# danielSanchezQ/dkg

Measured on AMD Instinct MI355X. Metric: verified shares/sec (whole node) at n=1024,t=511; full-ceremony wall time, higher is better.
Workload: dtype u32 (GF(2^255-19), Z_l); 1 GPU; one DKG ceremony n=1024, t=511 (share gen + round-2/4 checks + finalise); n=1024, t=511, parallelism=single GPU, verify_streams=2, rounds_2_4_fused=True, degree_split=4, recombination=short lattice multipliers, recombination_addends=affine Niels, stepping_additions=dedicated (complete redo where exceptional)

## Files before the change

dkg_amd/_lib.py:

```python
import ctypes
import os
import sys

HERE = os.path.dirname(os.path.abspath(__file__))
LIB_PATH = os.environ.get("DKG_AMD_LIB", os.path.join(HERE, "libdkg_amd.so"))

DKG_OK = 0
DKG_E_ARG = -1
DKG_E_DECODE = -2
DKG_E_DEVICE = -3
DKG_E_NOMEM = -4
REJECT, ACCEPT, SELF, SKIPPED, MISSING = 0, 1, 2, 3, 4
FIN_OK, FIN_R2_ERROR, FIN_R4_ERROR, FIN_PHASE4_ERROR, FIN_INSUFFICIENT, FIN_PANIC = 0, 1, 2, 3, 4, 5
COMPLAINT_IGNORED, COMPLAINT_NO_PHASE3 = 4, 5

_lib = None


class DkgError(RuntimeError):
    def __init__(self, code, msg=""):
        self.code = code
        names = {DKG_E_ARG: "DKG_E_ARG", DKG_E_DECODE: "DKG_E_DECODE", DKG_E_DEVICE: "DKG_E_DEVICE",
                 DKG_E_NOMEM: "DKG_E_NOMEM"}
        super().__init__(f"{names.get(code, code)}: {msg}")


class CeremonyOut(ctypes.Structure):
    _fields_ = [
        ("E", ctypes.c_void_p), ("A", ctypes.c_void_p),
        ("s", ctypes.c_void_p), ("s_prime", ctypes.c_void_p),
        ("dec2", ctypes.c_void_p), ("dec4", ctypes.c_void_p),
        ("qualified", ctypes.c_void_p), ("r2_error", ctypes.c_void_p), ("r4_error", ctypes.c_void_p),
        ("complaints2", ctypes.c_void_p), ("reconstruct", ctypes.c_void_p),
        ("final_share", ctypes.c_void_p), ("public_share", ctypes.c_void_p),
        ("mpk", ctypes.c_uint8 * 32),
        ("n_qualified", ctypes.c_int32), ("phase4_error", ctypes.c_int32),
        ("ms_round1", ctypes.c_double), ("ms_round2", ctypes.c_double), ("ms_round3", ctypes.c_double),
        ("ms_round4", ctypes.c_double), ("ms_finalise", ctypes.c_double), ("ms_total", ctypes.c_double),
    ]


class ShardOutcome(ctypes.Structure):
    _fields_ = [
        ("qualified", ctypes.c_void_p), ("complaints2", ctypes.c_void_p), ("r2_error", ctypes.c_void_p),
        ("reconstruct", ctypes.c_void_p), ("r4_error", ctypes.c_void_p),
        ("n_qualified", ctypes.c_int32), ("phase4_error", ctypes.c_int32),
    ]


class BatchOut(ctypes.Structure):
    _fields_ = [
        ("mpk", ctypes.c_void_p), ("n_qualified", ctypes.c_void_p), ("phase4_error", ctypes.c_void_p),
        ("qualified", ctypes.c_void_p),
        ("r2_error", ctypes.c_void_p), ("r4_error", ctypes.c_void_p), ("complaints2", ctypes.c_void_p),
        ("reconstruct", ctypes.c_void_p), ("final_share", ctypes.c_void_p), ("public_share", ctypes.c_void_p),
        ("dec2", ctypes.c_void_p), ("dec4", ctypes.c_void_p),
        ("ms_round1", ctypes.c_double), ("ms_checks", ctypes.c_double), ("ms_round3", ctypes.c_double),
        ("ms_finalise", ctypes.c_double), ("ms_total", ctypes.c_double),
    ]


def lib():
    global _lib
    if _lib is not None:
        return _lib
    if not os.path.exists(LIB_PATH):
        raise RuntimeError(f"{LIB_PATH} is missing: build it with `make -C dkg_amd` or __graft_entry__.build()")
    if "torch" not in sys.modules and not os.environ.get("DKG_NO_TORCH_PREIMPORT"):
        try:
            import torch
        except Exception:
            pass
    L = ctypes.CDLL(LIB_PATH)
    sz, p, u8p = ctypes.c_size_t, ctypes.c_void_p, ctypes.c_char_p
    L.dkg_ctx_create.argtypes = [ctypes.c_int, ctypes.POINTER(p)]
    L.dkg_ctx_destroy.argtypes = [p]
    L.dkg_ctx_destroy.restype = None
    L.dkg_ctx_last_error.argtypes = [p]
    L.dkg_ctx_last_error.restype = ctypes.c_char_p
    L.dkg_device_count.argtypes = []
    L.dkg_ctx_set_streams.argtypes = [p, ctypes.c_int]
    L.dkg_ctx_set_overlap.argtypes = [p, ctypes.c_int]
    L.dkg_ctx_set_verify_mode.argtypes = [p, ctypes.c_int]
    L.dkg_ctx_fallback_rows.argtypes = [p]
    L.dkg_ctx_fallback_rows.restype = sz
    L.dkg_ctx_set_split.argtypes = [p, ctypes.c_int]
    L.dkg_ctx_set_stepping.argtypes = [p, ctypes.c_int]
    L.dkg_ctx_set_field_mode.argtypes = [p, ctypes.c_int]
    L.dkg_ctx_set_binomial.argtypes = [p, ctypes.c_int]
    L.dkg_ctx_set_check.argtypes = [p, ctypes.c_int]
    L.dkg_ctx_last_split.argtypes = [p]
    L.dkg_ctx_last_split_len.argtypes = [p]
    L.dkg_ctx_last_split_len.restype = sz
    L.dkg_split_model_ms.argtypes = [sz, sz, sz, ctypes.c_int]
    L.dkg_split_model_ms.restype = ctypes.c_double
    L.dkg_split_len.argtypes = [sz, sz, sz, ctypes.c_int]
    L.dkg_split_len.restype = sz
    L.dkg_ctx_set_combine.argtypes = [p, ctypes.c_int]
    L.dkg_ctx_last_combine.argtypes = [p]
    L.dkg_ctx_last_binomial.argtypes = [p]
    L.dkg_ctx_set_addends.argtypes = [p, ctypes.c_int]
    L.dkg_ctx_set_stepping_formula.argtypes = [p, ctypes.c_int]
    L.dkg_ctx_stepping_redos.argtypes = [p]
    L.dkg_ctx_stepping_redos.restype = ctypes.c_longlong
    L.dkg_ctx_binomial_reruns.argtypes = [p]
    L.dkg_ctx_clock_probe.argtypes = [p, ctypes.c_uint, ctypes.POINTER(ctypes.c_double), ctypes.POINTER(ctypes.c_double)]
    L.dkg_device_pci_bus_id.argtypes = [ctypes.c_int, ctypes.c_char_p, ctypes.c_int]
    L.dkg_split_multipliers.argtypes = [sz, sz, ctypes.c_int, p, p]
    L.dkg_ctx_phase_ms.argtypes = [p, ctypes.c_char_p]
    L.dkg_ctx_phase_ms.restype = ctypes.c_double
    L.dkg_env_check.argtypes = [sz, sz]
    L.dkg_env_init.argtypes = [p, sz, sz, u8p, sz, p]
    L.dkg_msm_batch.argtypes = [p, sz, sz, u8p, u8p, p]
    L.dkg_fixed_base_batch.argtypes = [p, p, sz, u8p, p]
    L.dkg_poly_eval_batch.argtypes = [p, sz, sz, u8p, sz, p, p]
    L.dkg_points_valid_batch.argtypes = [p, sz, u8p, p]
    L.dkg_share_gen.argtypes = [p, sz, sz, sz, u8p, u8p, p, p, p, p]
    L.dkg_verify_pairs.argtypes = [p, sz, sz, ctypes.c_int, sz, sz, u8p, u8p, p, p]
    L.dkg_verify_receiver.argtypes = [p, sz, sz, ctypes.c_int, sz, u8p, u8p, p, p]
    L.dkg_ceremony_run.argtypes = [p, sz, sz, u8p, u8p, ctypes.POINTER(CeremonyOut)]
    L.dkg_ceremony_verify.argtypes = [p, sz, sz, u8p, u8p, u8p, u8p, ctypes.POINTER(CeremonyOut)]
    L.dkg_ceremony_verify_fetched.argtypes = [p, sz, sz, u8p, u8p, u8p, u8p, u8p, u8p, ctypes.POINTER(CeremonyOut)]
    L.dkg_ceremony_run_device.argtypes = [p, sz, sz, p, p, ctypes.POINTER(CeremonyOut)]
    L.dkg_ceremony_shard_device.argtypes = [p, sz, sz, sz, sz, p, p, p, p, p, p, ctypes.POINTER(ctypes.c_double)]
    L.dkg_ceremony_shard_verify_device.argtypes = [p, sz, sz, sz, sz, p, p, p, p, p, p, p, p,
                                                    ctypes.POINTER(ctypes.c_double)]
    L.dkg_ceremony_batch_device.argtypes = [p, sz, sz, sz, p, p, ctypes.POINTER(BatchOut)]
    L.dkg_ceremony_batch_verify.argtypes = [p, sz, sz, sz, u8p, u8p, u8p, u8p, ctypes.POINTER(BatchOut)]
    L.dkg_dealer_coeffs_device.argtypes = [p, u8p, ctypes.c_uint32, sz, sz, sz, sz, p, p]
    L.dkg_member_keys.argtypes = [p, u8p, ctypes.c_uint32, sz, p, p]
    L.dkg_enc_randomness.argtypes = [u8p, ctypes.c_uint32, sz, sz, sz, sz, p]
    L.dkg_enc_randomness_device.argtypes = [p, u8p, ctypes.c_uint32, sz, sz, sz, sz, sz, p]
    L.dkg_encrypt_shares.argtypes = [p, sz, sz, u8p, u8p, u8p, u8p, p, p]
    L.dkg_decrypt_shares.argtypes = [p, sz, sz, u8p, u8p, u8p, p, p, p]
    L.dkg_ceremony_run_full_device.argtypes = [p, sz, sz, p, p, p, u8p, u8p, ctypes.POINTER(CeremonyOut)]
    L.dkg_ceremony_verify_full.argtypes = [p, sz, sz, u8p, u8p, u8p, u8p, u8p, ctypes.POINTER(CeremonyOut)]
    L.dkg_member_keys_batch.argtypes = [p, u8p, ctypes.c_uint32, sz, sz, p, p]
    L.dkg_encrypt_shares_batch.argtypes = [p, sz, sz, u8p, u8p, u8p, u8p, p, p]
    L.dkg_decrypt_shares_batch.argtypes = [p, sz, sz, u8p, u8p, u8p, p, p, p]
    L.dkg_ceremony_batch_full_device.argtypes = [p, sz, sz, sz, p, p, p, u8p, u8p, ctypes.POINTER(BatchOut)]
    L.dkg_ceremony_batch_verify_full.argtypes = [p, sz, sz, sz, u8p, u8p, u8p, u8p, u8p, ctypes.POINTER(BatchOut),
                                                 p, p]
    L.dkg_ctx_set_batch_full_chunk.argtypes = [p, sz]
    L.dkg_misbehaviour_prove.argtypes = [p, sz, u8p, u8p, u8p, p]
    L.dkg_complaint1_verify.argtypes = [p, sz, sz, p, u8p, u8p, u8p, u8p, p]
    L.dkg_complaint3_verify.argtypes = [p, sz, sz, p, u8p, u8p, u8p, u8p, p]
    L.dkg_complaints_prove.argtypes = [p, sz, u8p, u8p, u8p, p]
    L.dkg_complaints_verify.argtypes = [p, sz, sz, sz, p, p, u8p, u8p, u8p, u8p, u8p, p, p]
    L.dkg_ctx_set_complaint_eval.argtypes = [p, ctypes.c_int]
    L.dkg_ceremony_verify_full_complaints.argtypes = [p, sz, sz, u8p, u8p, u8p, u8p, u8p, u8p, sz, p, p, u8p,
                                                      ctypes.POINTER(CeremonyOut), p, p]
    L.dkg_complaints3_verify.argtypes = [p, sz, sz, sz, p, p, u8p, u8p, u8p, u8p, u8p, u8p, p, p]
    L.dkg_ceremony_verify_fetched_proven.argtypes = [p, sz, sz, u8p, u8p, u8p, u8p, u8p, u8p, sz, p, p, u8p, u8p,
                                                     ctypes.POINTER(CeremonyOut), p, p, p]
    L.dkg_ceremony_verify_full_proven.argtypes = [p, sz, sz, u8p, u8p, u8p, u8p, u8p, u8p, sz, p, p, u8p, u8p, sz, p, p,
                                                  u8p, u8p, ctypes.POINTER(CeremonyOut), p, p, p, p, p]
    L.dkg_dealer_coeffs.argtypes = [u8p, ctypes.c_uint32, sz, sz, sz, p, p]
    L.dkg_scalar_sum_device.argtypes = [p, sz, sz, p, p, p]
    L.dkg_point_sum_device.argtypes = [p, sz, p, p, p]
    L.dkg_share_gen_device.argtypes = [p, sz, sz, sz, p, p, p, p, p, p]
    L.dkg_ceremony_shard_recon_device.argtypes = [p, sz, sz, sz, sz, u8p, u8p, u8p, u8p, p, p,
                                                  ctypes.POINTER(ctypes.c_int32)]
    L.dkg_finalise_parties.argtypes = [p, sz, sz, u8p, u8p, u8p, u8p, u8p, u8p, u8p, p, p, p]
    L.dkg_shard_range.argtypes = [sz, sz, sz, ctypes.POINTER(sz), ctypes.POINTER(sz)]
    L.dkg_shard_range.restype = None
    L.dkg_shard_rows.argtypes = [sz, sz]
    L.dkg_shard_rows.restype = sz
    L.dkg_shard_combine_device.argtypes = [p, sz, sz, sz, p, p, p, p, ctypes.POINTER(ShardOutcome)]
    L.dkg_shard_combine_packed_device.argtypes = [p, sz, sz, sz, p, p, p, p, ctypes.POINTER(ShardOutcome)]
    L.dkg_fixed_base_windows.argtypes = []
    L.dkg_key_comb_windows.argtypes = []
    L.dkg_packed_row_words.argtypes = [sz]
    L.dkg_packed_row_words.restype = sz
    L.dkg_decisions_pack_device.argtypes = [p, sz, sz, sz, sz, p, p]
    L.dkg_shard_finalise_device.argtypes = [p, sz, sz, sz, p, p, u8p, ctypes.c_int, p, p, p]
    L.dkg_multi_create.argtypes = [ctypes.POINTER(ctypes.c_int), ctypes.c_int, ctypes.POINTER(p)]
    L.dkg_multi_destroy.argtypes = [p]
    L.dkg_multi_destroy.restype = None
    L.dkg_multi_size.argtypes = [p]
    L.dkg_multi_ctx.argtypes = [p, ctypes.c_int]
    L.dkg_multi_ctx.restype = p
    L.dkg_multi_last_error.argtypes = [p]
    L.dkg_multi_last_error.restype = ctypes.c_char_p
    L.dkg_multi_phase_ms.argtypes = [p, ctypes.c_char_p]
    L.dkg_multi_phase_ms.restype = ctypes.c_double
    L.dkg_multi_env_init.argtypes = [p, sz, sz, u8p, sz, p]
    L.dkg_multi_ceremony_run.argtypes = [p, sz, sz, u8p, u8p, ctypes.POINTER(CeremonyOut)]
    L.dkg_multi_ceremony_run_device.argtypes = [p, sz, sz, ctypes.POINTER(p), ctypes.POINTER(p),
                                                ctypes.POINTER(CeremonyOut)]
    L.dkg_multi_ceremony_verify.argtypes = [p, sz, sz, u8p, u8p, u8p, u8p, ctypes.POINTER(CeremonyOut)]
    _lib = L
    return L


EXPORTED = [
    "dkg_ctx_create", "dkg_ctx_destroy", "dkg_ctx_last_error", "dkg_ctx_phase_ms", "dkg_ctx_set_streams", "dkg_ctx_set_overlap",
    "dkg_device_count", "dkg_env_init",
    "dkg_env_check", "dkg_msm_batch", "dkg_fixed_base_batch", "dkg_poly_eval_batch",
    "dkg_points_valid_batch", "dkg_share_gen", "dkg_verify_pairs", "dkg_verify_receiver",
    "dkg_ctx_set_split", "dkg_ctx_set_stepping", "dkg_ctx_set_field_mode", "dkg_ctx_set_binomial", "dkg_ctx_set_check", "dkg_ctx_last_split", "dkg_ctx_last_split_len", "dkg_ctx_set_verify_mode", "dkg_ctx_fallback_rows", "dkg_split_model_ms", "dkg_split_len",
    "dkg_ctx_set_combine", "dkg_ctx_last_combine", "dkg_ctx_last_binomial", "dkg_ctx_set_addends", "dkg_ctx_set_stepping_formula", "dkg_ctx_stepping_redos", "dkg_ctx_binomial_reruns", "dkg_split_multipliers",
    "dkg_ctx_clock_probe", "dkg_device_pci_bus_id",
    "dkg_ceremony_run", "dkg_ceremony_verify", "dkg_ceremony_verify_fetched", "dkg_ceremony_run_device", "dkg_ceremony_shard_device",
    "dkg_ceremony_shard_verify_device",
    "dkg_ceremony_batch_device", "dkg_ceremony_batch_verify", "dkg_member_keys", "dkg_enc_randomness",
    "dkg_enc_randomness_device", "dkg_encrypt_shares", "dkg_decrypt_shares", "dkg_ceremony_run_full_device",
    "dkg_ceremony_verify_full", "dkg_misbehaviour_prove", "dkg_complaint1_verify", "dkg_complaint3_verify", "dkg_dealer_coeffs", "dkg_dealer_coeffs_device",
    "dkg_scalar_sum_device", "dkg_point_sum_device", "dkg_ceremony_shard_recon_device", "dkg_finalise_parties",
    "dkg_share_gen_device", "dkg_shard_range", "dkg_shard_rows", "dkg_shard_combine_device",
    "dkg_shard_combine_packed_device", "dkg_packed_row_words", "dkg_fixed_base_windows", "dkg_key_comb_windows", "dkg_decisions_pack_device",
    "dkg_shard_finalise_device", "dkg_multi_create", "dkg_multi_destroy", "dkg_multi_size", "dkg_multi_ctx",
    "dkg_multi_last_error", "dkg_multi_phase_ms", "dkg_multi_env_init", "dkg_multi_ceremony_run",
    "dkg_multi_ceremony_run_device", "dkg_multi_ceremony_verify",
    "dkg_member_keys_batch", "dkg_encrypt_shares_batch", "dkg_decrypt_shares_batch", "dkg_ceremony_batch_full_device",
    "dkg_ceremony_batch_verify_full", "dkg_ctx_set_batch_full_chunk",
    "dkg_complaints_prove", "dkg_complaints_verify", "dkg_ctx_set_complaint_eval", "dkg_ceremony_verify_full_complaints",
    "dkg_complaints3_verify", "dkg_ceremony_verify_fetched_proven", "dkg_ceremony_verify_full_proven",
]
```

dkg_amd/csrc/ge25519.h:

```cpp
#pragma once
#include "fe25519.h"

struct ge_p3 {
  fe X, Y, Z, T;
};
struct ge_cached {
  fe YpX, YmX, Z2, T2d;
};
struct ge_aff {
  fe ypx, ymx, xy2d;
};

namespace ge_const {
__device__ static const uint32_t D[10] = {0x35978a3u, 0xd37284u, 0x3156ebdu, 0x6a0a0eu, 0x1c029u,
                                          0x179e898u, 0x3a03cbbu, 0x1ce7198u, 0x2e2b6ffu, 0x1480db3u};
__device__ static const uint32_t D2[10] = {0x2b2f159u, 0x1a6e509u, 0x22add7au, 0xd4141du, 0x38052u,
                                           0xf3d130u, 0x3407977u, 0x19ce331u, 0x1c56dffu, 0x901b67u};
__device__ static const uint32_t SQRT_M1[10] = {0x20ea0b0u, 0x186c9d2u, 0x8f189du, 0x35697fu,
                                                0xbd0c60u, 0x1fbd7a7u, 0x2804c9eu, 0x1e16569u,
                                                0x4fc1du, 0xae0c92u};
__device__ static const uint32_t SQRT_AD_MINUS_ONE[10] = {
    0x17b2e1bu, 0x1fda812u, 0x297afd2u, 0x60dbc2u, 0x2be7638u,
    0x1f5d1fdu, 0x27e6498u, 0x11581e7u, 0x3f2b834u, 0xdda4c6u};
__device__ static const uint32_t INVSQRT_A_MINUS_D[10] = {
// ... 150 lines not shown
    fe_dbl(c, c);
    fe_add(h, a, b);
    fe_sub(e, h, t);
    fe_sub(g, a, b);
    fe_add(f, c, g);
    fe_carry(f, f);
    fe_mul2(r.X, e, f, r.Y, g, h);
    if (with_t) fe_mul2(r.Z, g, f, r.T, e, h);
    else fe_mul(r.Z, g, f);
    return;
  }
  fe a, b, c, e, f, g, h, t;
  fe_sq(a, p.X);
  fe_sq(b, p.Y);
  fe_sq(c, p.Z);
  fe_dbl(c, c);
  fe_add(t, p.X, p.Y);
  fe_sq(t, t);
  fe_add(h, a, b);
  fe_sub(e, h, t);
  fe_sub(g, a, b);
  fe_add(f, c, g);
  fe_carry(f, f);
  fe_mul(r.X, e, f);
  fe_mul(r.Y, g, h);
  fe_mul(r.Z, g, f);
  if (with_t) fe_mul(r.T, e, h);
}

template <bool IL = false>
DKG_DEV void ge_dbl_rt(ge_p3& r, const ge_p3& p, bool with_t) {
  if constexpr (IL && DKG_PW) {
    fe a, b, c, t, h, e, g;
    fe_add(t, p.X, p.Y);
    fe_sq2(a, p.X, b, p.Y);
    fe_sq2(c, p.Z, t, t);
    fe_dbl(c, c);
    fe_add(h, a, b);
    fe_sub(e, h, t);
    fe_sub(g, a, b);
    fe_add(c, c, g);
    fe_carry(c, c);
    fe_mul2(r.X, e, c, r.Y, g, h);
    if (with_t) fe_mul2(r.Z, g, c, r.T, e, h);
    else fe_mul(r.Z, g, c);
    return;
  }
  fe a, b, c, t, h, e, g;
  fe_sq(a, p.X);
  fe_sq(b, p.Y);
  fe_sq(c, p.Z);
  fe_dbl(c, c);
  fe_add(t, p.X, p.Y);
  fe_sq(t, t);
  fe_add(h, a, b);
  fe_sub(e, h, t);
  fe_sub(g, a, b);
  fe_add(c, c, g);
  fe_carry(c, c);
  fe_mul(r.X, e, c);
  fe_mul(r.Y, g, h);
  fe_mul(r.Z, g, c);
  if (with_t) fe_mul(r.T, e, h);
}

template <bool IL = false>
DKG_DEV void ge_dbl_lean(ge_p3& r, const ge_p3& p, bool with_t) {
  if constexpr (IL && DKG_PW) {
    fe a, b, t, h, g;
    fe_sq2(a, p.X, b, p.Y);
    fe_add(h, a, b);
    fe_sub(g, a, b);
    fe_add(a, p.X, p.Y);
    fe_sq2(t, p.Z, a, a);
    fe_dbl(t, t);
    fe_add(t, t, g);
    fe_carry(t, t);
    fe_sub(b, h, a);
    fe_mul2(r.X, b, t, r.Y, g, h);
    if (with_t) fe_mul2(r.Z, g, t, r.T, b, h);
    else fe_mul(r.Z, g, t);
    return;
  }
  fe a, b, t, h, g;
  fe_sq(a, p.X);
  fe_sq(b, p.Y);
  fe_add(h, a, b);
  fe_sub(g, a, b);
  fe_sq(t, p.Z);
  fe_dbl(t, t);
  fe_add(t, t, g);
  fe_carry(t, t);
  fe_add(a, p.X, p.Y);
  fe_sq(a, a);
  fe_sub(b, h, a);
  fe_mul(r.X, b, t);
  fe_mul(r.Y, g, h);
  fe_mul(r.Z, g, t);
  if (with_t) fe_mul(r.T, b, h);
}

template <bool IL = false>
DKG_DEV void ge_add_signed(ge_p3& r, const ge_p3& p, const ge_cached& q, bool neg, bool with_t = true) {
  fe a, b, e, h, t, qa, qb;
#pragma unroll
  for (int i = 0; i < 10; i++) {
    qa.v[i] = neg ? q.YpX.v[i] : q.YmX.v[i];
    qb.v[i] = neg ? q.YmX.v[i] : q.YpX.v[i];
  }
  if constexpr (IL && DKG_PW) {
    fe u;
    fe_sub(t, p.Y, p.X);
    fe_add(u, p.Y, p.X);
    fe_mul2(a, t, qa, b, u, qb);
  } else {
    fe_sub(t, p.Y, p.X);
    fe_mul(a, t, qa);
    fe_add(t, p.Y, p.X);
    fe_mul(b, t, qb);
  }
  fe_sub(e, b, a);
  fe_add(h, b, a);
  if constexpr (IL && DKG_PW) {
    fe_mul2(a, p.T, q.T2d, b, p.Z, q.Z2);
  } else {
    fe_mul(a, p.T, q.T2d);
    fe_mul(b, p.Z, q.Z2);
  }
  fe na;
  fe_neg(na, a);
  fe_cmov(a, na, neg);
  fe_sub(t, b, a);
  fe_add(b, b, a);
  if constexpr (IL && DKG_PW) {
    fe_mul2(r.X, e, t, r.Y, b, h);
    if (with_t) fe_mul2(r.Z, b, t, r.T, e, h);
    else fe_mul(r.Z, b, t);
  } else {
    fe_mul(r.X, e, t);
    fe_mul(r.Y, b, h);
    fe_mul(r.Z, b, t);
    if (with_t) fe_mul(r.T, e, h);
  }
}

template <bool IL = false>
DKG_DEV void ge_madd_signed(ge_p3& r, const ge_p3& p, const ge_aff& q, bool neg, bool with_t = true) {
  fe a, b, e, h, t, qa, qb;
#pragma unroll
  for (int i = 0; i < 10; i++) {
    qa.v[i] = neg ? q.ypx.v[i] : q.ymx.v[i];
    qb.v[i] = neg ? q.ymx.v[i] : q.ypx.v[i];
  }
  if constexpr (IL && DKG_PW) {
    fe u;
    fe_sub(t, p.Y, p.X);
    fe_add(u, p.Y, p.X);
    fe_mul2(a, t, qa, b, u, qb);
  } else {
    fe_sub(t, p.Y, p.X);
    fe_mul(a, t, qa);
    fe_add(t, p.Y, p.X);
    fe_mul(b, t, qb);
  }
  fe_sub(e, b, a);
  fe_add(h, b, a);
  fe_mul(a, p.T, q.xy2d);
  fe na;
  fe_neg(na, a);
  fe_cmov(a, na, neg);
  fe_dbl(b, p.Z);
  fe_carry(b, b);
  fe_sub(t, b, a);
  fe_add(b, b, a);
  if constexpr (IL && DKG_PW) {
    fe_mul2(r.X, e, t, r.Y, b, h);
    if (with_t) fe_mul2(r.Z, b, t, r.T, e, h);
    else fe_mul(r.Z, b, t);
  } else {
    fe_mul(r.X, e, t);
    fe_mul(r.Y, b, h);
    fe_mul(r.Z, b, t);
    if (with_t) fe_mul(r.T, e, h);
  }
}


DKG_DEV bool fe_sqrt_ratio_m1(fe& r, const fe& u, const fe& v) {
  fe v3, v7, t, chk, neg_u, neg_u_i, sqrtm1;
  fe_ld(sqrtm1, ge_const::SQRT_M1);
  fe_sq(v3, v);
  fe_mul(v3, v3, v);
  fe_sq(v7, v3);
  fe_mul(v7, v7, v);
  fe_mul(t, u, v7);
  fe_pow22523(t, t);
  fe_mul(t, t, v3);
  fe_mul(r, t, u);
  fe_sq(chk, r);
  fe_mul(chk, chk, v);
  fe_neg(neg_u, u);
  fe_carry(neg_u, neg_u);
  fe_mul(neg_u_i, neg_u, sqrtm1);
  fe d;
  fe_sub(d, chk, u);
  bool correct = fe_iszero(d);
  fe_sub(d, chk, neg_u);
  bool flipped = fe_iszero(d);
  fe_sub(d, chk, neg_u_i);
  bool flipped_i = fe_iszero(d);
  fe r_prime;
  fe_mul(r_prime, r, sqrtm1);
  fe_cmov(r, r_prime, flipped || flipped_i);
  fe_abs(r, r);
  return correct || flipped;
}

DKG_DEV void fe_sq_x2(fe (&r)[2], const fe (&a)[2]) { fe_sq2(r[0], a[0], r[1], a[1]); }
DKG_DEV void fe_mul_x2(fe (&r)[2], const fe (&a)[2], const fe (&b)[2]) {
  fe_mul2(r[0], a[0], b[0], r[1], a[1], b[1]);
}
DKG_DEV void fe_sqn_x2(fe (&r)[2], const fe (&a)[2], int n) {
  fe_sq_x2(r, a);
  for (int i = 1; i < n; i++) fe_sq_x2(r, r);
}
DKG_DEV void fe_pow22523_x2(fe (&out)[2], const fe (&z)[2]) {
  fe t0[2], t1[2], t2[2];
  fe_sq_x2(t0, z);
  fe_sqn_x2(t1, t0, 2);
  fe_mul_x2(t1, z, t1);
  fe_mul_x2(t0, t0, t1);
  fe_sq_x2(t0, t0);
  fe_mul_x2(t0, t1, t0);
  fe_sqn_x2(t1, t0, 5);
  fe_mul_x2(t0, t1, t0);
  fe_sqn_x2(t1, t0, 10);
  fe_mul_x2(t1, t1, t0);
  fe_sqn_x2(t2, t1, 20);
  fe_mul_x2(t1, t2, t1);
  fe_sqn_x2(t1, t1, 10);
  fe_mul_x2(t0, t1, t0);
  fe_sqn_x2(t1, t0, 50);
  fe_mul_x2(t1, t1, t0);
  fe_sqn_x2(t2, t1, 100);
  fe_mul_x2(t1, t2, t1);
  fe_sqn_x2(t1, t1, 50);
  fe_mul_x2(t0, t1, t0);
  fe_sqn_x2(t0, t0, 2);
  fe_mul_x2(out, t0, z);
}
DKG_DEV void fe_invsqrt_x2(fe (&r)[2], const fe (&v)[2]) {
  fe v3[2], t[2];
  fe_sq_x2(v3, v);
  fe_mul_x2(v3, v3, v);
  fe_sq_x2(t, v3);
  fe_mul_x2(t, t, v);
  fe_pow22523_x2(t, t);
  fe_mul_x2(r, t, v3);
  fe chk[2];
  fe_sq_x2(chk, r);
  fe_mul_x2(chk, chk, v);
  fe sqrtm1, one, neg_one, neg_i;
  fe_ld(sqrtm1, ge_const::SQRT_M1);
  fe_one(one);
  fe_neg(neg_one, one);
  fe_carry(neg_one, neg_one);
  fe_mul(neg_i, neg_one, sqrtm1);
#pragma unroll
  for (int k = 0; k < 2; k++) {
    fe d, r_prime;
    fe_sub(d, chk[k], neg_one);
    const bool flipped = fe_iszero(d);
    fe_sub(d, chk[k], neg_i);
    const bool flipped_i = fe_iszero(d);
    fe_mul(r_prime, r[k], sqrtm1);
    fe_cmov(r[k], r_prime, flipped || flipped_i);
    fe_abs(r[k], r[k]);
  }
}

DKG_DEV bool ristretto_decode(ge_p3& p, const uint32_t (&w)[8]) {
  fe s;
  fe_frombytes32(s, w);
  uint32_t chk[8];
  fe_tobytes32(chk, s);
  uint32_t diff = 0;
#pragma unroll
  for (int i = 0; i < 8; i++) diff |= chk[i] ^ w[i];
  bool ok = (diff == 0) && ((w[0] & 1u) == 0);
  fe ss, u1, u2, u2sq, v, one, t, inv, den_x, den_y, dd;
  fe_one(one);
  fe_sq(ss, s);
  fe_sub(u1, one, ss);
  fe_carry(u1, u1);
  fe_add(u2, one, ss);
  fe_carry(u2, u2);
  fe_sq(u2sq, u2);
  fe_ld(dd, ge_const::D);
  fe_sq(t, u1);
  fe_mul(t, t, dd);
  fe_add(t, t, u2sq);
  fe_carry(t, t);
  fe_neg(v, t);
  fe_carry(v, v);
  fe_mul(t, v, u2sq);
  bool was_sq = fe_sqrt_ratio_m1(inv, one, t);
// ... 131 lines not shown
```

dkg_amd/csrc/host_crypto.h:

```cpp
#pragma once
#include <stddef.h>
#include <stdint.h>

namespace dkgh {

void blake2b(uint8_t* out, size_t outlen, const uint8_t* in, size_t inlen);
void chacha20(const uint8_t key[32], uint64_t block, uint8_t* out, size_t len);
void chacha20_ietf_xor(uint8_t* out, const uint8_t* in, size_t len, const uint8_t key[32], const uint8_t nonce[12]);

struct Zl {
  uint64_t w[4];
};
Zl zl_from_bytes_wide(const uint8_t* in, size_t len);
Zl zl_from_bits(const uint8_t in[32]);
Zl zl_from_u64(uint64_t x);
void zl_to_bytes(uint8_t out[32], const Zl& a);
Zl zl_add(const Zl& a, const Zl& b);
Zl zl_sub(const Zl& a, const Zl& b);
Zl zl_mul(const Zl& a, const Zl& b);
Zl zl_inv(const Zl& a);
bool zl_is_zero(const Zl& a);

bool short_multipliers(const Zl& y, int K, uint8_t (*mag)[32], int8_t* sign);

}
```

dkg_amd/csrc/kernels.hip:

```cpp
#ifdef DKG_FE_ILP
#define dkgk dkgk_ilp
#endif
#include "kernels.h"
#include "split.h"

#include <algorithm>
#include <cmath>
#include "points.h"

namespace dkgk {

constexpr int COMB_WORDS = AFF_WORDS * COMB_ENTRIES;

#ifndef DKG_DECODE_WAVES
#define DKG_DECODE_WAVES 2
#endif
__global__ __launch_bounds__(256, DKG_DECODE_WAVES) void k_decode(const uint32_t* __restrict__ comp, size_t count,
                                                uint32_t* __restrict__ ext, size_t stride,
                                                uint8_t* __restrict__ ok, size_t pm_N, size_t pm_npad,
                                                uint32_t nseg, uint32_t seg, size_t pm_L, size_t pm_pstride) {
  size_t e = (size_t)blockIdx.x * blockDim.x + threadIdx.x;
  if (e >= count) return;
  uint32_t w[8];
  ld_words8(w, comp + 8 * e);
// ... 1319 lines not shown
        ld_z(z, R, Rz, pt(i));
        fe_mul(acc, acc, z);
      }
    }
  }
  fe inv;
  fe_invert(inv, acc);
  fe d2;
  fe_ld(d2, ge_const::D2);
#pragma unroll 1
  for (int b = nblk - 1; b >= 0; b--) {
    fe z[AFF_BLK], q[AFF_BLK];
    static_assert(AFF_BLK >= 2, "q[1] = z[0] below");
#pragma unroll
    for (int k = 0; k < AFF_BLK; k++) {
      if (AFF_BLK * b + k < cnt) ld_z(z[k], R, Rz, pt(AFF_BLK * b + k));
      else fe_one(z[k]);
    }
    fe_copy(q[1], z[0]);
#pragma unroll
    for (int k = 2; k < AFF_BLK; k++) fe_mul(q[k], q[k - 1], z[k - 1]);
    fe blk, ib;
    fe_mul(blk, q[AFF_BLK - 1], z[AFF_BLK - 1]);
    {
      const uint4* a4 = reinterpret_cast<const uint4*>(A + pt(AFF_BLK * b) * AFFP_WORDS);
      const uint4 q0 = a4[0], q1 = a4[1], q2 = a4[2];
      const fe pre = {{q0.x, q0.y, q0.z, q0.w, q1.x, q1.y, q1.z, q1.w, q2.x, q2.y}};
      fe_mul(ib, inv, pre);
    }
    fe_mul(inv, inv, blk);
    auto point = [&](auto kc) {
      constexpr int k = decltype(kc)::value;
      const int i = AFF_BLK * b + k;
      fe zi;
      if constexpr (k > 0) {
        fe_mul(zi, ib, q[k]);
        fe_mul(ib, ib, z[k]);
      } else {
        fe_copy(zi, ib);
      }
      if (i < cnt) {
        ge_p3 p;
        pt_load_aos(p, R, pt(i));
        fe x, y;
        fe_mul(x, p.X, zi);
        fe_mul(y, p.Y, zi);
        fe_mul(p.T, p.T, zi);
        fe_mul(p.T, p.T, d2);
        fe_add(p.X, y, x);
        fe_sub(p.Y, y, x);
        st_fe3(A + pt(i) * AFFP_WORDS, p.X, p.Y, p.T);
      }
    };
    for_desc<AFF_BLK>(point);
  }
}

void affine_pieces(size_t width, size_t pstride, size_t pieces, size_t nrecv, const uint32_t* R, uint32_t* A,
                   hipStream_t stream, const uint32_t* Rz, size_t j0, size_t jn) {
  if (!jn) jn = nrecv - j0;
  if (!width || !jn || !pieces) return;
  unsigned ls = 32;
  while (ls > 1 && (size_t)(ls / 2) * AFF_RUN >= jn) ls /= 2;
  const size_t runs = (jn + (size_t)ls * AFF_RUN - 1) / ((size_t)ls * AFF_RUN), lanes = pieces * width * runs * ls;
  hipLaunchKernelGGL(k_affine_pieces, dim3((unsigned)((lanes + 255) / 256)), dim3(256), 0, stream, width, pstride,
                     pieces, nrecv, R, A, Rz, j0, jn, ls);
}

template <int U, int K, int KL>
DKG_DEV void aff_addends(uint32_t* qs, ge_aff* qr, const uint32_t* A, size_t pstride, size_t cc, size_t nrecv,
                         size_t j) {
  if constexpr (U < K) {
    const uint4* a4 = reinterpret_cast<const uint4*>(A + (((size_t)U * pstride + cc) * nrecv + j) * AFFP_WORDS);
    uint32_t w[AFFP_WORDS];
#pragma unroll
    for (int k = 0; k < AFFP_WORDS / 4; k++) {
      const uint4 v = a4[k];
      w[4 * k] = v.x;
      w[4 * k + 1] = v.y;
      w[4 * k + 2] = v.z;
      w[4 * k + 3] = v.w;
    }
    if constexpr (U < KL) {
      uint32_t* s = qs + U * AFF_WORDS * 64 + threadIdx.x;
#pragma unroll
      for (int k = 0; k < AFF_WORDS; k++) s[k * 64] = w[k];
    } else {
#pragma unroll
      for (int i = 0; i < 10; i++) {
        qr[U - KL].ypx.v[i] = w[i];
        qr[U - KL].ymx.v[i] = w[10 + i];
        qr[U - KL].xy2d.v[i] = w[20 + i];
      }
    }
    aff_addends<U + 1, K, KL>(qs, qr, A, pstride, cc, nrecv, j);
  }
}
template <int U, int K, int KL>
DKG_DEV void aff_position(ge_p3& acc, uint64_t w, const uint32_t* qs, const ge_aff* qr, bool last) {
  if constexpr (U < K) {
    const int e = (int8_t)(w >> (8 * U));
    if (e != 0) {
      const bool t = last || higher_digits64<U, K>(w);
      if constexpr (U < KL) ge_madd_lds<DKG_AFF_IL != 0>(acc, acc, qs + U * AFF_WORDS * 64 + threadIdx.x, e < 0, 64, t);
      else ge_madd_signed<DKG_AFF_IL != 0>(acc, acc, qr[U - KL], e < 0, t);
    }
    aff_position<U + 1, K, KL>(acc, w, qs, qr, last);
  }
}

template <int K, int KL>
__global__ __launch_bounds__(64, K == 2 ? 3 : 2) void k_combine_aff(size_t width, size_t pstride, size_t nrecv,
                                                      const uint32_t* __restrict__ digits,
                                                      const int16_t* __restrict__ top,
                                                      const uint32_t* __restrict__ A, uint32_t* __restrict__ R,
                                                      size_t j0) {
  __shared__ uint32_t qs[KL * AFF_WORDS * 64];
  const size_t c = (size_t)blockIdx.x * 64 + threadIdx.x;
  const size_t j = j0 + blockIdx.y;
  const bool live = c < width;
  const size_t cc = live ? c : 0;
  ge_aff qr[K - KL > 0 ? K - KL : 1];
  aff_addends<0, K, KL>(qs, qr, A, pstride, cc, nrecv, j);
  const uint32_t* dw = digits + j * 256;
  const uint32_t* dw1 = digits + (nrecv + j) * 256;
  const int tp = top[j];
  ge_p3 acc;
  ge_identity(acc);
#pragma unroll 1
  for (int b = tp; b >= 0; b--) {
    uint64_t w = (uint32_t)__builtin_amdgcn_readfirstlane(dw[b]);
    if constexpr (K > 4) w |= (uint64_t)(uint32_t)__builtin_amdgcn_readfirstlane(dw1[b]) << 32;
    if (b != tp) ge_dbl_lean<DKG_AFF_IL != 0>(acc, acc, w != 0 || b == 0);
    aff_position<0, K, KL>(acc, w, qs, qr, b == 0);
  }
  if (live) pt_store_aos<DKG_COMB_NT != 0>(R, c * nrecv + j, acc);
}

void combine_short_aff(size_t width, size_t pstride, size_t pieces, size_t nrecv, const uint32_t* digits,
                       const int16_t* top, const uint32_t* A, uint32_t* R, hipStream_t stream, size_t j0, size_t jn) {
  if (!jn) jn = nrecv - j0;
  if (!width || !jn || pieces < 2 || pieces > 5) return;
  const dim3 grid((unsigned)((width + 63) / 64), (unsigned)jn);
  if (pieces == 2)
    hipLaunchKernelGGL((k_combine_aff<2, 1>), grid, dim3(64), 0, stream, width, pstride, nrecv, digits, top, A, R, j0);
  else if (pieces == 3)
    hipLaunchKernelGGL((k_combine_aff<3, 2>), grid, dim3(64), 0, stream, width, pstride, nrecv, digits, top, A, R, j0);
  else if (pieces == 4)
    hipLaunchKernelGGL((k_combine_aff<4, 2>), grid, dim3(64), 0, stream, width, pstride, nrecv, digits, top, A, R, j0);
  else
    hipLaunchKernelGGL((k_combine_aff<5, 2>), grid, dim3(64), 0, stream, width, pstride, nrecv, digits, top, A, R, j0);
}

void combine(size_t width, size_t pstride, size_t pieces, size_t nrecv, const int8_t* digits, const int16_t* top,
             uint32_t* R, hipStream_t stream) {
  if (!width || !nrecv || pieces < 2) return;
  const dim3 grid((unsigned)((width + 63) / 64), (unsigned)nrecv);
  if (pieces == 2)
    hipLaunchKernelGGL(k_combine<1>, grid, dim3(64), 0, stream, width, pstride, (int)pieces, nrecv, digits, top, R);
  else
    hipLaunchKernelGGL(k_combine<2>, grid, dim3(64), 0, stream, width, pstride, (int)pieces, nrecv, digits, top, R);
}

__global__ __launch_bounds__(256, DKG_COMB_WAVES) void k_check(size_t ndealers, size_t nrecv, size_t dealer_base, size_t recv_base,
                                               uint32_t nmod, int round,
                                               const uint32_t* __restrict__ s, const uint32_t* __restrict__ sp,
                                               const uint32_t* __restrict__ R,
                                               const uint32_t* __restrict__ tab_g,
                                               const uint32_t* __restrict__ tab_h,
                                               const uint8_t* __restrict__ dok, uint8_t* __restrict__ dec,
                                               const uint32_t* __restrict__ scale) {
  const size_t p = (size_t)blockIdx.x * blockDim.x + threadIdx.x;
  if (p >= ndealers * nrecv) return;
  const size_t i = p / nrecv, j = p % nrecv;
  ge_p3 acc, r;
  ge_identity(acc);
  sc x, f;
  if (scale) sc_load(f, scale + 8 * j);
  sc_load(x, s + 8 * p);
  if (scale) sc_mont_mul(x, x, f);
  combw_mul_add(acc, x, tab_g);
  if (round == 2) {
    sc_load(x, sp + 8 * p);
    if (scale) sc_mont_mul(x, x, f);
    combw_mul_add(acc, x, tab_h);
  }
  pt_load_aos(r, R, p);
  const bool eq = ristretto_eq(acc, r);
  uint8_t v = dok[i] ? (eq ? 1 : 0) : (round == 2 ? 4 : 0);
  if ((uint32_t)((i + dealer_base) % nmod) == (uint32_t)(j + recv_base)) v = 2;
  dec[p] = v;
}

void check(size_t ndealers, size_t nrecv, size_t dealer_base, size_t recv_base, size_t nmod, int round,
           const uint32_t* s, const uint32_t* sp, const uint32_t* R, const uint32_t* tab_g,
           const uint32_t* tab_h, const uint8_t* dok, uint8_t* dec, hipStream_t stream, const uint32_t* scale) {
  const size_t total = ndealers * nrecv;
  if (!total) return;
  hipLaunchKernelGGL(k_check, dim3((unsigned)((total + 255) / 256)), dim3(256), 0, stream, ndealers, nrecv,
                     dealer_base, recv_base, (uint32_t)nmod, round, s, sp, R, tab_g, tab_h, dok, dec, scale);
}

template <int PASS>
__global__ __launch_bounds__(256, DKG_COMB_WAVES) void k_check_both(size_t ndealers, size_t nrecv, size_t dealer0, size_t dealer_base,
                                                    uint32_t nmod, const uint32_t* __restrict__ s,
                                                    const uint32_t* __restrict__ sp, const uint32_t* __restrict__ R,
                                                    const uint32_t* __restrict__ tab_g,
                                                    const uint32_t* __restrict__ tab_h,
                                                    const uint8_t* __restrict__ dok, uint8_t* __restrict__ dec2,
                                                    uint8_t* __restrict__ dec4, const uint32_t* __restrict__ scale,
                                                    size_t j0, size_t jn, uint32_t* __restrict__ accb) {
  const size_t p = (size_t)blockIdx.x * blockDim.x + threadIdx.x;
  if (p >= ndealers * jn) return;
  const size_t i = dealer0 + p / jn, j = j0 + p % jn;
  const size_t cE = (i / 64) * 128 + i % 64, cA = cE + 64;
  const size_t q = i * nrecv + j;
  const bool self = (uint32_t)((i + dealer_base) % nmod) == (uint32_t)j;
  ge_p3 acc, r;
  sc x, f;
  if (scale) sc_load(f, scale + 8 * j);
  if constexpr (PASS != 2) {
    ge_identity(acc);
    sc_load(x, s + 8 * q);
    if (scale) sc_mont_mul(x, x, f);
    combw_mul_add<DKG_CHECK_IL != 0>(acc, x, tab_g);
    pt_load_aos(r, R, cA * nrecv + j);
    const bool eq = ristretto_eq(acc, r);
    dec4[q] = self ? 2 : ((dok[cA] && eq) ? 1 : 0);
    if constexpr (PASS == 1) {
      pt_store_aos(accb, p, acc);
      return;
    }
  } else {
    pt_load_aos(acc, accb, p);
  }
  sc_load(x, sp + 8 * q);
  if (scale) sc_mont_mul(x, x, f);
  combw_mul_add<DKG_CHECK_IL != 0>(acc, x, tab_h);
  pt_load_aos(r, R, cE * nrecv + j);
  const bool eq = ristretto_eq(acc, r);
  dec2[q] = self ? 2 : (dok[cE] ? (eq ? 1 : 0) : 4);
}

void check_both(size_t ndealers, size_t nrecv, size_t dealer0, size_t dealer_base, size_t nmod, const uint32_t* s,
                const uint32_t* sp, const uint32_t* R, const uint32_t* tab_g, const uint32_t* tab_h,
                const uint8_t* dok, uint8_t* dec2, uint8_t* dec4, hipStream_t stream, const uint32_t* scale, size_t j0,
                size_t jn, uint32_t* acc) {
  if (!jn) jn = nrecv - j0;
  const size_t total = ndealers * jn;
  if (!total) return;
  const dim3 grid((unsigned)((total + 255) / 256));
  if (!acc) {
    hipLaunchKernelGGL(k_check_both<0>, grid, dim3(256), 0, stream, ndealers, nrecv, dealer0, dealer_base,
                       (uint32_t)nmod, s, sp, R, tab_g, tab_h, dok, dec2, dec4, scale, j0, jn, acc);
    return;
  }
  hipLaunchKernelGGL(k_check_both<1>, grid, dim3(256), 0, stream, ndealers, nrecv, dealer0, dealer_base,
                     (uint32_t)nmod, s, sp, R, tab_g, tab_h, dok, dec2, dec4, scale, j0, jn, acc);
  hipLaunchKernelGGL(k_check_both<2>, grid, dim3(256), 0, stream, ndealers, nrecv, dealer0, dealer_base,
                     (uint32_t)nmod, s, sp, R, tab_g, tab_h, dok, dec2, dec4, scale, j0, jn, acc);
}

__global__ void k_fill_all_identity(size_t S, uint32_t* __restrict__ out) {
  const size_t e = (size_t)blockIdx.x * blockDim.x + threadIdx.x;
  if (e >= S) return;
  ge_p3 id;
  ge_identity(id);
  pt_store(out, S, e, id);
}

void fill_identity(size_t S, uint32_t* out, hipStream_t stream) {
  if (!S) return;
  hipLaunchKernelGGL(k_fill_all_identity, dim3((unsigned)((S + 255) / 256)), dim3(256), 0, stream, S, out);
}

__global__ void k_dealer_ok(size_t ndealers, size_t N, const uint8_t* __restrict__ pok, uint8_t* __restrict__ ok) {
  const size_t i = (size_t)blockIdx.x * blockDim.x + threadIdx.x;
  if (i >= ndealers) return;
  uint8_t v = 1;
  for (size_t k = 0; k < N; k++) v &= pok[i * N + k];
  ok[i] = v;
}

__global__ void k_and_dealer_mask(size_t D, uint32_t nseg, uint32_t seg, const uint8_t* __restrict__ extra,
                                  uint8_t* __restrict__ dok) {
  const size_t i = (size_t)blockIdx.x * blockDim.x + threadIdx.x;
  if (i >= D) return;
  const size_t col = (i / 64) * 64 * nseg + seg * 64 + i % 64;
  dok[col] &= extra[i];
}

void and_dealer_mask(size_t D, int nseg, int seg, const uint8_t* extra, uint8_t* dok, hipStream_t stream) {
  if (!D) return;
  hipLaunchKernelGGL(k_and_dealer_mask, dim3((unsigned)((D + 255) / 256)), dim3(256), 0, stream, D, (uint32_t)nseg,
                     (uint32_t)seg, extra, dok);
}

__global__ __launch_bounds__(256) void k_mask_not_and(size_t V, const uint8_t* __restrict__ a,
                                                      const uint8_t* __restrict__ b, uint8_t* __restrict__ out) {
  const size_t i = (size_t)blockIdx.x * 256 + threadIdx.x;
  if (i < V) out[i] = !a[i] && (!b || b[i]);
}

void mask_not_and(size_t V, const uint8_t* a, const uint8_t* b, uint8_t* out, hipStream_t stream) {
  if (!V) return;
  hipLaunchKernelGGL(k_mask_not_and, dim3((unsigned)((V + 255) / 256)), dim3(256), 0, stream, V, a, b, out);
// ... 507 lines not shown
```

dkg_amd/csrc/kernels_decl.inc:

```
namespace dkgk {

void decode_points(const uint32_t* comp, size_t count, uint32_t* ext, size_t stride, uint8_t* ok,
                   hipStream_t stream);
void place_position_major(const uint32_t* src, size_t sstride, size_t D, size_t N, size_t npad, uint32_t* out,
                          hipStream_t stream, int nseg = 1, int seg = 0, size_t L = 0, size_t pstride = 0);
void gather_points(const uint32_t* src, size_t sstride, size_t step, size_t k0, size_t count, uint32_t* dst,
                   size_t dstride, hipStream_t stream);
void decode_position_major(const uint32_t* comp, size_t D, size_t N, size_t npad, uint32_t* out, uint8_t* ok,
                           hipStream_t stream, int nseg = 1, int seg = 0, size_t L = 0, size_t pstride = 0);
void fill_identity(size_t S, uint32_t* out, hipStream_t stream);
void check_both(size_t ndealers, size_t nrecv, size_t dealer0, size_t dealer_base, size_t nmod, const uint32_t* s,
                const uint32_t* sp, const uint32_t* R, const uint32_t* tab_g, const uint32_t* tab_h,
                const uint8_t* dok, uint8_t* dec2, uint8_t* dec4, hipStream_t stream, const uint32_t* scale = nullptr,
                size_t j0 = 0, size_t jn = 0, uint32_t* acc = nullptr);
void encode_points(const uint32_t* ext, size_t stride, size_t count, uint32_t* comp, hipStream_t stream);
void build_comb(const uint32_t* ext, size_t stride, size_t e0, uint32_t* tab, hipStream_t stream, size_t count = 1);
void build_combw(const uint32_t* ext, size_t stride, size_t e0, uint32_t* tab, hipStream_t stream, size_t count = 1);

void commit_position_major(size_t D, size_t N, const uint32_t* a, const uint32_t* b, const uint32_t* tab_g,
                           const uint32_t* tab_h, uint32_t* out, size_t W, size_t L, size_t pstride, uint32_t* A0,
                           size_t A0stride, hipStream_t stream);
void commit(size_t count, const uint32_t* a, const uint32_t* b, const uint32_t* tab_g,
            const uint32_t* tab_h, uint32_t* A_ext, uint32_t* E_ext, hipStream_t stream, size_t stride = 0);
void share_eval(size_t D, size_t n, size_t N, const uint32_t* a, const uint32_t* b, uint32_t* s,
                uint32_t* sp, hipStream_t stream);
void poly_eval(size_t D, size_t N, const uint32_t* coeffs, size_t M, const uint32_t* xs, uint32_t* out,
               hipStream_t stream);

uint32_t* binomial(size_t width, size_t npad, size_t N, const uint32_t* C, uint32_t* e0, uint32_t* e1,
                   hipStream_t stream, size_t pieces = 1, size_t pstride = 0, size_t last_len = 0);
void binom_init(size_t width, size_t npad, size_t N, const uint32_t* C, uint32_t* e0, hipStream_t stream,
                size_t pieces = 1, size_t pstride = 0);
void binom_step(size_t r, size_t width, size_t npad, size_t N, const uint32_t* C, const uint32_t* in, uint32_t* out,
                hipStream_t stream, size_t pieces = 1, size_t pstride = 0, size_t last_len = 0,
                uint32_t* flags = nullptr, size_t col_base = 0, size_t dreal = 0, unsigned gw = 64,
                bool flag_any = false,
                bool nt = false,
                bool il = false);
void binomial_wave_redo(size_t width, size_t npad, size_t N, const uint32_t* C, uint32_t* e, hipStream_t stream,
                        size_t pieces, size_t pstride, size_t last_len, uint32_t* flags, size_t col_base,
                        size_t dreal, unsigned gw);
uint32_t* binomial_wave(size_t width, size_t npad, size_t N, const uint32_t* C, uint32_t* e, hipStream_t stream,
                        size_t pieces = 1, size_t pstride = 0, size_t last_len = 0, uint32_t* eT = nullptr,
                        bool prefetch = false, uint32_t* flags = nullptr, size_t col_base = 0, size_t dreal = 0,
                        unsigned gw = 64);
void binom_step_pair(size_t r, size_t width, size_t npad, size_t N, const uint32_t* C, const uint32_t* in,
                     uint32_t* out, hipStream_t stream, size_t pieces = 1, size_t pstride = 0, size_t last_len = 0);
void to_column_major(size_t width, size_t npad, size_t N, const uint32_t* e, uint32_t* eT, size_t pieces,
                     size_t pstride, hipStream_t stream);
struct StepShape {
  size_t nblk, P, per, bs, maxbs;
};
StepShape stepping_shape(size_t N);
double step_occupancy(size_t bs, size_t maxbs);
bool stepping_whole_columns(size_t L, size_t pieces, size_t last_len);
double stepping_cycles(size_t cols, size_t N, size_t pieces, size_t last_len, bool whole);
double stepping_waves_per_simd(size_t cols, size_t N, size_t pieces, size_t last_len, bool whole);
size_t stepping_flag_words(size_t ndealers, size_t pieces);
bool stepping(size_t ndealers, size_t npad, size_t N, const uint32_t* e, size_t nrecv, uint32_t* R,
              uint32_t* stream_a, uint32_t* stream_b, hipStream_t stream, size_t pieces = 1, size_t pstride = 0,
              size_t last_len = 0, bool whole = true, uint32_t* flags = nullptr, size_t col0 = 0,
              size_t dreal = (size_t)-1, unsigned gw = 64, uint32_t* Rz = nullptr, uint32_t* tail_a = nullptr,
              uint32_t* tail_b = nullptr);
int stepping_tail_phases(size_t N, size_t nrecv, size_t pieces);
size_t stepping_tail_words(size_t ndealers, size_t N);
void combine(size_t width, size_t pstride, size_t pieces, size_t nrecv, const int8_t* digits, const int16_t* top,
             uint32_t* R, hipStream_t stream);
void combine_short(size_t width, size_t pstride, size_t pieces, size_t nrecv, const uint32_t* digits,
                   const int16_t* top, uint32_t* R, hipStream_t stream);
void affine_pieces(size_t width, size_t pstride, size_t pieces, size_t nrecv, const uint32_t* R, uint32_t* A,
                   hipStream_t stream, const uint32_t* Rz = nullptr, size_t j0 = 0, size_t jn = 0);
void combine_short_aff(size_t width, size_t pstride, size_t pieces, size_t nrecv, const uint32_t* digits,
                       const int16_t* top, const uint32_t* A, uint32_t* R, hipStream_t stream, size_t j0 = 0,
                       size_t jn = 0);
void check(size_t ndealers, size_t nrecv, size_t dealer_base, size_t recv_base, size_t nmod, int round,
           const uint32_t* s, const uint32_t* sp, const uint32_t* R, const uint32_t* tab_g,
           const uint32_t* tab_h, const uint8_t* dealer_ok, uint8_t* decision, hipStream_t stream,
           const uint32_t* scale = nullptr);
void and_dealer_mask(size_t D, int nseg, int seg, const uint8_t* extra, uint8_t* dok, hipStream_t stream);
void dealer_ok(size_t ndealers, size_t N, const uint8_t* point_ok, uint8_t* ok, hipStream_t stream);
void horner(size_t ndealers, size_t npad, size_t N, const uint32_t* C, uint32_t x0, size_t nrecv, uint32_t* R,
            hipStream_t stream);
void sum_points(size_t count, const uint32_t* pts, size_t stride, const uint8_t* mask, uint32_t* out, size_t ostride,
                size_t col, hipStream_t stream, size_t groups = 1);
void add_points(size_t count, const uint32_t* a, const uint32_t* b, size_t stride, uint32_t* out, hipStream_t stream);
void r4_error(size_t groups, size_t n, size_t t, const uint8_t* dec, const uint8_t* qmask, uint8_t* out,
              hipStream_t stream);
void decision_summary(size_t groups, size_t n, const uint8_t* dec, uint8_t* row_reject, int32_t* complaints,
                      hipStream_t stream);
void apply_skipped(size_t groups, size_t n, uint8_t* dec, const uint8_t* qmask, hipStream_t stream);
void compact_ranks(size_t n, size_t ws, size_t R, size_t width, const void* in, void* out, hipStream_t stream);
void mask_not_and(size_t V, const uint8_t* a, const uint8_t* b, uint8_t* out, hipStream_t stream);
void row_reject(size_t rows, size_t n, const uint8_t* dec, uint8_t* out, hipStream_t stream);
size_t key_comb_words();
int key_comb_windows();
void build_key_combs(const uint32_t* ext, size_t stride, size_t e0, uint32_t* tab, hipStream_t stream,
                     size_t count);
int fixed_base_windows();
void pack_rows(size_t rows, size_t nvalid, size_t n, size_t d0, const uint8_t* dec, uint32_t* out, uint32_t* err,
               hipStream_t stream);
void unpack_ranks(size_t n, size_t ws, size_t R, const uint32_t* in, uint8_t* out, hipStream_t stream);
void from_uniform(const uint32_t* in16, uint32_t* out, hipStream_t stream);

void msm_batch(size_t B, size_t N, const uint32_t* scalars, const uint32_t* pts, size_t stride, uint32_t* tab,
               uint32_t* out_ext, hipStream_t stream);
void fixed_base(size_t count, const uint32_t* scalars, const uint32_t* tab, uint32_t* out_ext,
                hipStream_t stream);
void to_position_major(size_t D, size_t N, size_t npad, const uint32_t* in, uint32_t* out,
                       hipStream_t stream);
void reduce_scalars(size_t count, const uint32_t* in, uint32_t* out, hipStream_t stream);
void sum_shares(size_t D, size_t n, const uint32_t* s, const uint8_t* mask, uint32_t* out, hipStream_t stream,
                size_t groups = 1);
void dealer_coeffs(size_t rows, size_t D, size_t d0, uint32_t c0, const uint32_t* master, size_t N, uint32_t* seeds,
                   uint32_t* a, uint32_t* b, hipStream_t stream);

void enc_mul(size_t D, size_t n, const uint32_t* r, const uint32_t* tab_gw, const uint32_t* tabs_pk, uint32_t* R_ext,
             uint32_t* K_ext, hipStream_t stream);
void dec_mul(size_t D, size_t n, const uint32_t* sk, const uint32_t* R_ext, uint32_t* K_ext, hipStream_t stream,
             uint32_t* table = nullptr);
size_t dec_mul_table_words(size_t D, size_t n);
void sym_xor(size_t D, size_t n, const uint32_t* Kc, bool decrypt, uint32_t* ct, uint32_t* s, uint32_t* sp,
             hipStream_t stream);
void dealer_seeds(size_t rows, size_t D, size_t d0, uint32_t c0, const uint32_t* master, uint32_t* seeds,
                  hipStream_t stream);
void enc_randomness(size_t rows, size_t n, size_t N, const uint32_t* seeds, uint32_t* r, hipStream_t stream);

size_t benc_tab_words();
void benc_tab(size_t keys, const uint32_t* pk_ext, size_t stride, uint32_t* tab, hipStream_t stream);
void benc_mul(size_t keys, size_t n, const uint32_t* r, const uint32_t* tab, uint32_t* K_ext, size_t count,
              hipStream_t stream);
size_t bdec_mul_table_words(size_t keys, size_t n);
size_t bdec_launch_waves();
void bdec_mul(size_t keys, size_t n, const uint32_t* sk, const uint32_t* R_ext, uint32_t* K_ext, size_t count,
              uint32_t* table, hipStream_t stream);

size_t cmp_ladder_table_words(size_t cnt);
void cmp_ladder(size_t cnt, bool joint, const uint32_t* bp, const uint32_t* bq, const uint32_t* sa, const uint32_t* sb,
                const uint32_t* Pext, size_t pstride, uint32_t* T, uint32_t* out, hipStream_t stream);
void cmp_horner(size_t cnt, const uint32_t* list, const uint32_t* accuser, const uint32_t* accused, const uint32_t* Eext,
                size_t stride, size_t N, int nb, uint32_t* R, hipStream_t stream);
void cv_prep(size_t C, const uint32_t* accuser, const uint32_t* pk, const uint32_t* enc, const uint32_t* proofs,
             uint32_t* Pc, uint32_t* rs, uint32_t* nc, uint32_t* p12, uint32_t* bp1, uint32_t* bp2, uint32_t* bq2,
             hipStream_t stream);
void cv_check(size_t C, const uint32_t* accuser, const uint32_t* p12, const uint32_t* ridx, const uint32_t* Rh,
              const uint32_t* Rt, const uint32_t* scale, const uint32_t* tab_g, const uint32_t* tab_h, uint8_t* eq,
              hipStream_t stream);
void cv_final(size_t C, const uint32_t* accuser, const uint32_t* accused, const uint32_t* pk, const uint32_t* enc,
              const uint32_t* proofs, const uint32_t* a1c, const uint32_t* a2c, const uint8_t* pok, const uint8_t* rowok,
              const uint8_t* fetched, const uint8_t* eq, int32_t* verdict, hipStream_t stream);
void cp_prep(size_t C, const uint32_t* sk, const uint32_t* enc, const uint32_t* w, uint32_t* Pc, uint32_t* ls,
             uint32_t* lb, uint32_t* gs, hipStream_t stream);
void cp_finish(size_t C, const uint32_t* enc, const uint32_t* lc, const uint32_t* gc, const uint32_t* gs,
               uint32_t* proofs, hipStream_t stream);
void qualified_complaints(size_t rows, size_t n, const uint8_t* dec, const uint8_t* cmask, uint8_t* rej, uint8_t* qmask,
                          hipStream_t stream);
void c3_prep(size_t C, size_t n, const uint32_t* accuser, const uint32_t* accused, const uint32_t* share,
             const uint32_t* randomness, uint32_t* sr, uint32_t* acc2, uint32_t* acd2, hipStream_t stream);
void c3_check(size_t C, const uint32_t* accuser, const uint32_t* sr, const uint32_t* ridx, const uint32_t* Rh,
              const uint32_t* Rt, const uint32_t* scale, const uint32_t* tab_g, const uint32_t* tab_h, uint8_t* eq,
              hipStream_t stream);
void c3_final(size_t C, size_t n, const uint32_t* accused, const uint8_t* rowok, const uint8_t* qualified,
              const uint8_t* fetched3, const uint8_t* eq, int32_t* verdict, hipStream_t stream);

void interp(size_t D, size_t N, size_t nrecv, const uint32_t* WT, const uint32_t* s, const uint32_t* sp, uint32_t* F,
            uint32_t* Fp, hipStream_t stream);
void coef_check(size_t D, size_t N, const uint32_t* F, const uint32_t* Fp, const uint32_t* Eext, const uint32_t* Aext,
                size_t cstride, const uint32_t* tab_g, const uint32_t* tab_h, uint8_t* okE, uint8_t* okA,
                hipStream_t stream);
void interp_decide(size_t D, size_t nrecv, size_t N, size_t dealer_base, size_t nmod, const uint32_t* s,
                   const uint32_t* sp, const uint32_t* F, const uint32_t* Fp, const uint8_t* dokE, const uint8_t* dokA,
                   const uint8_t* cE, const uint8_t* cA, const uint32_t* tab_g, const uint32_t* tab_h, uint8_t* dec2,
                   uint8_t* dec4, hipStream_t stream);
void and_mask(size_t D, const uint8_t* extra, uint8_t* ok, hipStream_t stream);

}
```

dkg_amd/csrc/lattice.cpp:

```cpp
#include <math.h>
#include <string.h>

#include "host_crypto.h"

namespace dkgh {
namespace {

struct I512 {
  uint64_t w[8];
};
typedef unsigned __int128 u128;

I512 i_zero() {
  I512 r;
  memset(r.w, 0, sizeof r.w);
  return r;
}
bool i_neg_p(const I512& a) { return (a.w[7] >> 63) != 0; }
I512 i_neg(const I512& a) {
  I512 r;
  u128 c = 1;
  for (int i = 0; i < 8; i++) {
    c += (u128)(~a.w[i]);
    r.w[i] = (uint64_t)c;
    c >>= 64;
  }
  return r;
}
I512 i_sub(const I512& a, const I512& b) {
  I512 r;
  u128 bb = 0;
  for (int i = 0; i < 8; i++) {
    const u128 d = (u128)a.w[i] - b.w[i] - bb;
    r.w[i] = (uint64_t)d;
    bb = (d >> 64) & 1;
  }
  return r;
}
I512 i_mul_shift(const I512& a, int64_t m, int e) {
  const bool neg = m < 0;
  const uint64_t um = neg ? (uint64_t)0 - (uint64_t)m : (uint64_t)m;
  I512 r;
  u128 c = 0;
  for (int i = 0; i < 8; i++) {
    c += (u128)a.w[i] * um;
    r.w[i] = (uint64_t)c;
    c >>= 64;
  }
  if (e > 0) {
    const int wl = e / 64, bl = e % 64;
    I512 s = i_zero();
    for (int i = 7; i >= wl; i--) {
      uint64_t v = r.w[i - wl] << bl;
      if (bl && i - wl - 1 >= 0) v |= r.w[i - wl - 1] >> (64 - bl);
      s.w[i] = v;
    }
    r = s;
  }
  return neg ? i_neg(r) : r;
}
int i_bits(const I512& a) {
  const I512 m = i_neg_p(a) ? i_neg(a) : a;
  for (int i = 7; i >= 0; i--)
    if (m.w[i]) return 64 * i + 64 - __builtin_clzll(m.w[i]);
  return 0;
}
long double i_ld(const I512& a) {
  const bool neg = i_neg_p(a);
  const I512 m = neg ? i_neg(a) : a;
  static const long double P64[8] = {1.0L, 0x1p64L, 0x1p128L, 0x1p192L, 0x1p256L, 0x1p320L, 0x1p384L, 0x1p448L};
  int t = 7;
  while (t > 0 && !m.w[t]) t--;
  const long double v = t > 0 ? ((long double)m.w[t] * P64[1] + (long double)m.w[t - 1]) * P64[t - 1]
                              : (long double)m.w[0];
  return neg ? -v : v;
}
I512 i_add(const I512& a, const I512& b) {
  I512 r;
  u128 c = 0;
  for (int i = 0; i < 8; i++) {
    c += (u128)a.w[i] + b.w[i];
    r.w[i] = (uint64_t)c;
    c >>= 64;
  }
  return r;
}
void i_naf_shape(const I512& a, int& len, int& weight) {
  const I512 m = i_neg_p(a) ? i_neg(a) : a;
  const I512 m3 = i_add(m, i_add(m, m));
  len = 0;
  weight = 0;
  for (int i = 0; i < 8; i++) {
    const uint64_t h = (m3.w[i] >> 1) | (i < 7 ? m3.w[i + 1] << 63 : 0);
    const uint64_t x = (m3.w[i] ^ m.w[i]) >> 1 | (i < 7 ? (m3.w[i + 1] ^ m.w[i + 1]) << 63 : 0);
    weight += __builtin_popcountll(x);
    if (h) len = 64 * i + 64 - __builtin_clzll(h);
  }
}
double chain_cost(const I512* v, int K) {
  int top = 0, adds = 0;
  for (int u = 0; u < K; u++) {
    int len, w;
    i_naf_shape(v[u], len, w);
    top = top > len ? top : len;
    adds += w;
  }
  return (top > 0 ? top - 1 : 0) * 1815.0 + adds * 2002.0;
}

I512 i_from_zl(const Zl& z) {
  I512 r = i_zero();
  for (int i = 0; i < 4; i++) r.w[i] = z.w[i];
  return r;
}
Zl zl_of(const I512& a) {
  const bool neg = i_neg_p(a);
  const I512 m = neg ? i_neg(a) : a;
  uint8_t b[64];
  for (int i = 0; i < 64; i++) b[i] = (uint8_t)(m.w[i / 8] >> (8 * (i % 8)));
  const Zl z = zl_from_bytes_wide(b, 64);
  return neg ? zl_sub(zl_from_u64(0), z) : z;
}

const int KMAX = 5;

void sub_multiple(I512* v, const I512* vj, int K, long double q) {
  if (q == 0) return;
  int e;
  const long double fr = frexpl(q, &e);
  int64_t m;
  int sh;
  if (e <= 62) {
    m = (int64_t)q;
    sh = 0;
  } else {
    m = (int64_t)ldexpl(fr, 62);
    sh = e - 62;
  }
  for (int u = 0; u < K; u++) v[u] = i_sub(v[u], i_mul_shift(vj[u], m, sh));
}

void gram_schmidt(const I512 (*B)[KMAX], int K, long double (*mu)[KMAX], long double* nrm) {
  long double bs[KMAX][KMAX];
  for (int i = 0; i < K; i++) {
    long double bi[KMAX];
    for (int u = 0; u < K; u++) bs[i][u] = bi[u] = i_ld(B[i][u]);
    for (int j = 0; j < i; j++) {
      long double d = 0;
      for (int u = 0; u < K; u++) d += bi[u] * bs[j][u];
      mu[i][j] = nrm[j] > 0 ? d / nrm[j] : 0;
      for (int u = 0; u < K; u++) bs[i][u] -= mu[i][j] * bs[j][u];
    }
    long double s = 0;
    for (int u = 0; u < K; u++) s += bs[i][u] * bs[i][u];
    nrm[i] = s;
  }
}

}

bool short_multipliers(const Zl& y, int K, uint8_t (*mag)[32], int8_t* sign) {
  if (K < 2 || K > KMAX) return false;
  I512 B[KMAX][KMAX];
  Zl p = zl_from_u64(1), pw[KMAX];
  for (int u = 0; u < K; u++) {
    pw[u] = p;
    p = zl_mul(p, y);
  }
  I512 lv;
  {
    const uint64_t Lw[4] = {0x5812631a5cf5d3edull, 0x14def9dea2f79cd6ull, 0ull, 0x1000000000000000ull};
    lv = i_zero();
    for (int i = 0; i < 4; i++) lv.w[i] = Lw[i];
  }
  for (int u = 0; u < K; u++) B[0][u] = i_from_zl(pw[u]);
  for (int i = 1; i < K; i++)
    for (int u = 0; u < K; u++) B[i][u] = u == i ? lv : i_zero();
  long double mu[KMAX][KMAX], nrm[KMAX];
  int k = 1, guard = 0;
  while (k < K && guard++ < 4096) {
    for (int pass = 0; pass < 16; pass++) {
      gram_schmidt(B, K, mu, nrm);
      bool done = true;
      for (int j = k - 1; j >= 0; j--) {
        const long double q = roundl(mu[k][j]);
        if (q == 0) continue;
        done = false;
        sub_multiple(B[k], B[j], K, q);
        for (int i = 0; i < j; i++) mu[k][i] -= q * mu[j][i];
      }
      if (done) break;
    }
    gram_schmidt(B, K, mu, nrm);
    if (nrm[k] >= (0.99L - mu[k][k - 1] * mu[k][k - 1]) * nrm[k - 1]) {
      k++;
    } else {
      for (int u = 0; u < K; u++) {
        const I512 t = B[k][u];
        B[k][u] = B[k - 1][u];
        B[k - 1][u] = t;
      }
      k = k > 1 ? k - 1 : 1;
    }
  }
  const int CRMAX = 4, CR = K <= 4 ? 4 : 2;
  I512 mult[KMAX][2 * CRMAX + 1][KMAX];
  for (int i = 0; i < K; i++)
    for (int c = -CR; c <= CR; c++)
      for (int u = 0; u < K; u++) mult[i][c + CR][u] = i_mul_shift(B[i][u], c, 0);
  I512 v[KMAX];
  for (int u = 0; u < K; u++) v[u] = i_from_zl(pw[u]);
  double best = chain_cost(v, K);
  I512 win[KMAX];
  bool have = false;
  int ncomb = 1;
  for (int i = 0; i < K; i++) ncomb *= 2 * CR + 1;
  for (int code = 0; code < ncomb; code++) {
    int cf[KMAX], first = 0;
    for (int i = 0, cd = code; i < K; i++, cd /= 2 * CR + 1) {
      cf[i] = cd % (2 * CR + 1) - CR;
      if (!first && cf[i]) first = cf[i];
    }
    if (first <= 0) continue;
    I512 c[KMAX];
    bool small = true;
    for (int u = 0; u < K && small; u++) {
      c[u] = i_zero();
      for (int i = 0; i < K; i++)
        if (cf[i]) c[u] = i_add(c[u], mult[i][cf[i] + CR][u]);
      small = i_bits(c[u]) < 253;
    }
    if (!small) continue;
    const double cost = chain_cost(c, K);
    if (!(cost < best)) continue;
    if (zl_is_zero(zl_of(c[0]))) continue;
    best = cost;
    have = true;
    for (int u = 0; u < K; u++) win[u] = c[u];
  }
  if (have) {
    const Zl b = zl_of(win[0]);
    bool ok = true;
    for (int u = 1; u < K && ok; u++) ok = zl_is_zero(zl_sub(zl_of(win[u]), zl_mul(b, pw[u])));
    const bool flip = i_neg_p(win[0]);
    if (ok)
      for (int u = 0; u < K; u++) v[u] = flip ? i_neg(win[u]) : win[u];
  }
  for (int u = 0; u < K; u++) {
    sign[u] = i_neg_p(v[u]) ? -1 : 1;
    const I512 m = sign[u] < 0 ? i_neg(v[u]) : v[u];
    for (int i = 0; i < 32; i++) mag[u][i] = (uint8_t)(m.w[i / 8] >> (8 * (i % 8)));
  }
  return true;
}

}
```

dkg_amd/csrc/runtime.hip:

```cpp
#include <hip/hip_runtime.h>

#include <cstdio>
#include <cstdlib>
#include <cstring>
#include <algorithm>
#include <map>
#include <memory>
#include <string>
#include <thread>
#include <vector>

#include "../../include/dkg_amd.h"
#include "host_crypto.h"
#include "kernels.h"
#include "kernels_ilp.h"

struct dkg_ctx {
  int device = 0;
  hipStream_t stream = nullptr;
  std::string err;
  std::map<std::string, std::pair<void*, size_t>> bufs;
  std::map<std::string, std::pair<void*, size_t>> hbufs;
  uint32_t* tab_g = nullptr;
  uint32_t* tab_h = nullptr;
  uint32_t* tab_gw = nullptr;
  uint32_t* tab_hw = nullptr;
  uint8_t h[32] = {0};
  bool have_h = false;
  size_t threshold = 0, nr_members = 0;
  hipEvent_t ev[8] = {};
  hipEvent_t pev[5] = {};
  hipEvent_t hev[9] = {};
  int hy_timed = 0;
  static constexpr int MAX_SUB = 8;
  int nsub = 2;
  hipStream_t sub[MAX_SUB] = {};
  hipEvent_t fork = nullptr, join[MAX_SUB] = {};
  hipStream_t side = nullptr;
  hipEvent_t side_fork = nullptr, shares_done = nullptr, pub_done = nullptr;
  hipEvent_t terms_done = nullptr;
  bool shares_pending = false;
  bool overlap = true;
  int split = 0;
  std::vector<uint8_t> key_tabs_pk;
  uint8_t fb_base[32] = {0};
  bool fb_valid = false;
  int binom_mode = 0;
  int step_mode = 0;
  int check_mode = 0;
  int fe_mode = 0;
  int verify_mode = 0;
  size_t vinv_N = 0;
  size_t fallback_rows = 0;
  int last_split = 1;
  size_t last_split_len = 0;
  size_t ydig_n = 0, ydig_L = 0;
  int combine_mode = 0;
  int last_combine = 0;
  int last_binomial = 0;
  int step_formula = 0;
  uint32_t* last_step_flags = nullptr;
  size_t last_step_flag_words = 0;
  bool binom_step_ded = false;
  uint32_t* binom_any = nullptr;
  const uint32_t* binom_any_host = nullptr;
  int last_binom_rerun = 0;
  int addend_mode = 0;
  size_t sdig_n = 0, sdig_L = 0, sdig_K = 0;
  const uint32_t* last_R = nullptr;
  const uint32_t* last_scale = nullptr;
  const uint8_t* last_dok = nullptr;
  int complaint_eval = 0;
  const uint32_t* ext_E = nullptr;
  const uint32_t* ext_A = nullptr;
  const uint32_t* r1_a = nullptr;
  const uint32_t* r1_b = nullptr;
  size_t r1_D = 0;
  uint32_t* r1_A0 = nullptr;
  size_t ext_stride = 0;
  const uint32_t* shard_s = nullptr;
  size_t shard_n = 0, shard_d0 = 0, shard_D = 0;
  size_t bfull_chunk = 0;
  std::vector<hipEvent_t> bf_pool;
  std::vector<std::pair<int, hipEvent_t>> bf_marks;
  std::string timed_tag;
  std::map<std::string, double> phase_ms;
};

namespace {

constexpr size_t PTB = 160;
constexpr size_t PT_WORDS_H = 40;
constexpr size_t AFFP_WORDS_H = 32;
constexpr size_t COMB_BYTES = 30 * 512 * 4;
#ifndef DKG_COMBW_BITS
#define DKG_COMBW_BITS 19
#endif
constexpr size_t COMBW_BYTES =
    (size_t)(256 / DKG_COMBW_BITS + 1) * (1u << (DKG_COMBW_BITS - 1)) * 32 * 4;
const uint8_t BASEPOINT[32] = {0xe2, 0xf2, 0xae, 0x0a, 0x6a, 0xbc, 0x4e, 0x71, 0xa8, 0x84, 0xa9,
                               0x61, 0xc5, 0x00, 0x51, 0x5f, 0x58, 0xe3, 0x0b, 0x6a, 0xa5, 0x82,
                               0xdd, 0x8d, 0xb6, 0xa6, 0x59, 0x45, 0xe0, 0x8d, 0x2d, 0x76};

struct Fail {
  int code;
};

#define HCK(call)                                                                      \
  do {                                                                                 \
    hipError_t e_ = (call);                                                            \
    if (e_ != hipSuccess) {                                                            \
      ctx->err = std::string(#call) + ": " + hipGetErrorString(e_);                    \
      throw Fail{DKG_E_DEVICE};                                                        \
    }                                                                                  \
  } while (0)

template <typename T = void>
T* buf(dkg_ctx* ctx, const char* name, size_t bytes) {
  if (bytes == 0) bytes = 16;
  auto it = ctx->bufs.find(name);
  if (it != ctx->bufs.end() && it->second.second >= bytes) return reinterpret_cast<T*>(it->second.first);
  if (it != ctx->bufs.end()) {
    HCK(hipDeviceSynchronize());
    HCK(hipFree(it->second.first));
    ctx->bufs.erase(it);
  }
  void* p = nullptr;
  hipError_t e = hipMalloc(&p, bytes);
  if (e != hipSuccess) {
    ctx->err = std::string("hipMalloc(") + name + ", " + std::to_string(bytes) + "): " + hipGetErrorString(e);
    throw Fail{DKG_E_NOMEM};
  }
  ctx->bufs[name] = {p, bytes};
  return reinterpret_cast<T*>(p);
}

template <typename T = void>
T* hbuf(dkg_ctx* ctx, const char* name, size_t bytes) {
  if (bytes == 0) bytes = 16;
  auto it = ctx->hbufs.find(name);
  if (it != ctx->hbufs.end() && it->second.second >= bytes) return reinterpret_cast<T*>(it->second.first);
  if (it != ctx->hbufs.end()) {
    HCK(hipDeviceSynchronize());
    HCK(hipHostFree(it->second.first));
    ctx->hbufs.erase(it);
  }
  void* p = nullptr;
  hipError_t e = hipHostMalloc(&p, bytes, hipHostMallocDefault);
  if (e != hipSuccess) {
    ctx->err = std::string("hipHostMalloc(") + name + ", " + std::to_string(bytes) + "): " + hipGetErrorString(e);
    throw Fail{DKG_E_NOMEM};
  }
  ctx->hbufs[name] = {p, bytes};
  return reinterpret_cast<T*>(p);
}

void h2d(dkg_ctx* ctx, void* d, const void* h, size_t n) {
  if (n) HCK(hipMemcpyAsync(d, h, n, hipMemcpyHostToDevice, ctx->stream));
}
void d2h(dkg_ctx* ctx, void* h, const void* d, size_t n) {
  if (n) HCK(hipMemcpyAsync(h, d, n, hipMemcpyDeviceToHost, ctx->stream));
}
void sync(dkg_ctx* ctx) {
  HCK(hipStreamSynchronize(ctx->stream));
}
void check_launch(dkg_ctx* ctx) { HCK(hipGetLastError()); }

size_t pad64(size_t x) { return (x + 63) / 64 * 64; }

template <typename F>
int guarded(dkg_ctx* ctx, F&& f) {
  if (!ctx) return DKG_E_ARG;
  try {
    HCK(hipSetDevice(ctx->device));
    int rc = f();
    return rc;
  } catch (const Fail& x) {
    return x.code;
  } catch (const std::exception& x) {
    ctx->err = x.what();
    return DKG_E_NOMEM;
  }
}

void comb_for_point(dkg_ctx* ctx, const uint8_t p[32], uint32_t* tab, bool* ok, uint32_t* tab8 = nullptr) {
  uint32_t* comp = buf<uint32_t>(ctx, "comb_in", 32);
  uint32_t* ext = buf<uint32_t>(ctx, "comb_ext", PTB);
  uint8_t* okd = buf<uint8_t>(ctx, "comb_ok", 1);
  h2d(ctx, comp, p, 32);
  dkgk::decode_points(comp, 1, ext, 1, okd, ctx->stream);
  if (tab) dkgk::build_comb(ext, 1, 0, tab, ctx->stream);
  if (tab8) dkgk::build_combw(ext, 1, 0, tab8, ctx->stream);
  check_launch(ctx);
  uint8_t v = 0;
  d2h(ctx, &v, okd, 1);
  sync(ctx);
  *ok = v != 0;
}

uint32_t* upload_scalars(dkg_ctx* ctx, const char* name, const uint8_t* host, size_t count) {
  uint32_t* raw = buf<uint32_t>(ctx, "scalar_raw", 32 * count);
  uint32_t* red = buf<uint32_t>(ctx, name, 32 * count);
  h2d(ctx, raw, host, 32 * count);
  dkgk::reduce_scalars(count, raw, red, ctx->stream);
  return red;
}

#ifndef DKG_BINOM_NT_BYTES_DEFAULT
#define DKG_BINOM_NT_BYTES_DEFAULT 0.0
#endif
bool binom_nt(size_t r, size_t columns) {
  static const double lim = [] {
    const char* e = getenv("DKG_BINOM_NT_BYTES");
    return e ? atof(e) : DKG_BINOM_NT_BYTES_DEFAULT;
  }();
  return 2.0 * (double)(r + 1) * (double)columns * 160.0 > lim;
}

void collect_phases(dkg_ctx* ctx) {
  if (ctx->timed_tag.empty()) return;
  const char* names[4] = {"binomial", "stepping", "combine", "check"};
  for (int i = 0; i < 4; i++) {
    float ms = 0;
    HCK(hipEventElapsedTime(&ms, ctx->pev[i], ctx->pev[i + 1]));
    ctx->phase_ms[ctx->timed_tag + "." + names[i]] = ms;
  }
  ctx->timed_tag.clear();
}

struct VerifySeg {
  int round;
  size_t D, dealer_base;
  const uint32_t* Ccomp;
  const uint32_t* s;
  const uint32_t* sp;
  uint8_t* dec;
  const uint8_t* extra_ok = nullptr;
  size_t self_mod = 0;
};

#ifndef DKG_BINOM_PAIR_WAVES
#define DKG_BINOM_PAIR_WAVES 1.0
#endif
#ifndef DKG_BINOM_ILP_WAVES
#define DKG_BINOM_ILP_WAVES 1.5
#endif
#ifndef DKG_BINOM_IL_WAVES_DEFAULT
#define DKG_BINOM_IL_WAVES_DEFAULT 0.0
#endif
double binom_il_waves() {
  static const double v = [] {
    const char* e = getenv("DKG_BINOM_IL_WAVES");
    return e ? atof(e) : DKG_BINOM_IL_WAVES_DEFAULT;
  }();
  return v;
}
double binom_ilp_waves() {
  static const double v = [] {
    const char* e = getenv("DKG_BINOM_ILP_WAVES");
    return e ? atof(e) : DKG_BINOM_ILP_WAVES;
  }();
  return v;
}
#ifndef DKG_BINOM_WAVE_PF
#define DKG_BINOM_WAVE_PF 0
#endif
#ifndef DKG_BINOM_WAVE_DED
#define DKG_BINOM_WAVE_DED 1
#endif
#ifndef DKG_BINOM_STEP_DED
#define DKG_BINOM_STEP_DED 1
#endif
#ifndef DKG_BINOM_WAVE_COLMAJOR
#define DKG_BINOM_WAVE_COLMAJOR 0
#endif
#ifndef DKG_BINOM_WAVE_GROUPS
#define DKG_BINOM_WAVE_GROUPS 16384
#endif

bool use_ilp(const dkg_ctx* ctx, bool latency_bound) {
  return ctx->fe_mode == 2 || (ctx->fe_mode == 0 && latency_bound);
}

void wait_shares(dkg_ctx* ctx, hipStream_t st) {
  if (ctx->shares_pending) HCK(hipStreamWaitEvent(st, ctx->shares_done, 0));
}

size_t last_piece_len(size_t N, size_t U, size_t L) {
  return (U - 1) * L < N ? N - (U - 1) * L : L;
}

bool stepping_whole_pays(size_t cols, size_t U, size_t L, size_t Lr) {
  return dkgk::stepping_whole_columns(L, U, Lr) &&
         dkgk::stepping_cycles(cols, L, U, Lr, true) < 0.98 * dkgk::stepping_cycles(cols, L, U, Lr, false);
}

constexpr size_t SHORT_MAX = 5;
#ifndef DKG_AUTO_SHORT5
#define DKG_AUTO_SHORT5 0
#endif

double split_model_ms(size_t cols, size_t n, size_t N, size_t U, size_t L, bool short_mult) {
  const double DBL = 1000, ADD = 1400, SIMDS = 1024, THR = 4.5, LAT = 8, LAT_ILP = 6, LAUNCH = 3e-3 * 2.4e6;
  const size_t Lr = last_piece_len(N, U, L), off = L - Lr;
  auto cost = [&](size_t m) {
    uint64_t pos = 0, neg = 0;
    int len = 0;
    for (uint64_t v = m; v; v >>= 1, len++) {
      if (v & 1) {
        if ((v & 3) == 1) {
          pos |= 1ull << len;
          v -= 1;
        } else {
          neg |= 1ull << len;
          v += 1;
        }
      }
    }
    if (len >= 3 && !(((pos | neg) >> (len - 2)) & 1) && ((neg >> (len - 3)) & 1)) {
      pos = (pos & ~(1ull << (len - 1))) | (3ull << (len - 3));
      neg &= ~(1ull << (len - 3));
      len--;
    }
    const int nz = __builtin_popcountll(pos | neg);
    return ADD + (len > 1 ? (len - 1) * DBL + (nz - 1) * ADD : 0.0);
  };

  std::vector<double> pre(L + 1, 0.0);
  for (size_t m = 1; m <= L; m++) pre[m] = pre[m - 1] + cost(m);
  const double waves_col = (double)cols / 64;
  double cyc = 0;
  for (size_t r = 1; r < L; r++) {
    const double work = waves_col * ((U - 1) * pre[r] + (r > off ? pre[r - off] : 0.0)) * THR / SIMDS;
    const double lat = waves_col * U * (r + 1) / SIMDS < 1.5 ? LAT_ILP : LAT;
    cyc += work + cost(r) * lat + LAUNCH;
  }
  if (U > 1) {
    const double bits = 253.0 * (U - 1) / U;
    const double per = short_mult && U <= SHORT_MAX ? bits * 950 + U * bits / 3 * ADD
                                            : (U % 2 == 0 ? 253 * 950 + 85 * ADD : 0.0) +
                                                  ((U + 1) / 2 - 1) * (253 * 950 + 170 * ADD);
    const double waves = (double)cols / 64 * n;
    cyc += std::max(waves * per * THR / SIMDS, per * LAT);
  }
  cyc += n * ADD * dkgk::stepping_cycles(cols, L, U, Lr, stepping_whole_pays(cols, U, L, Lr));
  return cyc / 2.4e6;
}

size_t split_len(size_t cols, size_t n, size_t N, size_t U, bool short_mult = true) {
  const size_t L1 = (N + U - 1) / U;
  if (U == 1) return L1;
  const size_t L64 = (L1 + 63) / 64 * 64;
  if (L64 == L1 || (U - 1) * L64 >= N) return L1;
  return split_model_ms(cols, n, N, U, L64, short_mult) < split_model_ms(cols, n, N, U, L1, short_mult) ? L64 : L1;
}

double split_model_ms(size_t cols, size_t n, size_t N, size_t U, bool short_mult = true) {
  return split_model_ms(cols, n, N, U, split_len(cols, n, N, U, short_mult), short_mult);
}

size_t choose_split(dkg_ctx* ctx, size_t cols, size_t n, size_t N) {
  if (ctx->split > 0) return std::min<size_t>((size_t)ctx->split, N);
  const bool sm = ctx->combine_mode != 1;
  const double base = split_model_ms(cols, n, N, 1, sm);
  std::vector<double> ms(17, 0.0);
  double best_ms = base;
  size_t umax = 1;
  for (size_t U = 2; U <= 16; U++) {
    if (N < 64 * U) break;
    ms[U] = split_model_ms(cols, n, N, U, sm && (U <= 4 || (ctx->addend_mode == 0 && DKG_AUTO_SHORT5)));
    best_ms = std::min(best_ms, ms[U]);
    umax = U;
  }
  if (!(best_ms < 0.9 * base)) return 1;
  for (size_t U = 2; U <= umax; U++)
    if (ms[U] <= best_ms) return U;
  return 1;
}

void naf_digits(const uint8_t b[32], int8_t* d, int16_t* tp) {
  uint32_t k[9] = {0};
  for (int w = 0; w < 8; w++)
    k[w] = (uint32_t)b[4 * w] | (uint32_t)b[4 * w + 1] << 8 | (uint32_t)b[4 * w + 2] << 16 | (uint32_t)b[4 * w + 3] << 24;
  *tp = -1;
  for (int i = 0; i < 256; i++) {
    d[i] = 0;
    if (!((k[i >> 5] >> (i & 31)) & 1u)) continue;
    int8_t dg = 1;
    if ((k[(i + 1) >> 5] >> ((i + 1) & 31)) & 1u) {
      dg = -1;
      uint64_t carry = 1ull << (i & 31);
      for (int w = i >> 5; carry && w < 9; w++) {
        const uint64_t sum = (uint64_t)k[w] + carry;
        k[w] = (uint32_t)sum;
        carry = sum >> 32;
      }
    } else {
      k[i >> 5] &= ~(1u << (i & 31));
    }
    d[i] = dg;
    *tp = (int16_t)i;
  }
}

void split_digits(dkg_ctx* ctx, size_t n, size_t L, const int8_t** digits, const int16_t** top) {
  int8_t* dd = buf<int8_t>(ctx, "v.ydig", 512 * n);
  int16_t* dt = buf<int16_t>(ctx, "v.ytop", 4 * n);
  *digits = dd;
  *top = dt;
  if (ctx->ydig_n == n && ctx->ydig_L == L) return;
  std::vector<int8_t> hd(512 * n, 0);
  std::vector<int16_t> ht(2 * n, -1);
  for (size_t j = 0; j < n; j++) {
    dkgh::Zl x = dkgh::zl_from_u64(j + 1), y = dkgh::zl_from_u64(1);
    for (size_t e = L; e; e >>= 1) {
      if (e & 1) y = dkgh::zl_mul(y, x);
      x = dkgh::zl_mul(x, x);
    }
    uint8_t b[32];
    dkgh::zl_to_bytes(b, y);
    naf_digits(b, &hd[512 * j], &ht[2 * j]);
    dkgh::zl_to_bytes(b, dkgh::zl_mul(y, y));
    naf_digits(b, &hd[512 * j + 256], &ht[2 * j + 1]);
  }
  h2d(ctx, dd, hd.data(), hd.size());
  h2d(ctx, dt, ht.data(), 4 * n);
  ctx->ydig_n = n;
  ctx->ydig_L = L;
}

void short_vectors(size_t n, size_t L, size_t K, std::vector<uint8_t>& mag, std::vector<int8_t>& sign) {
  mag.assign(n * K * 32, 0);
  sign.assign(n * K, 1);
  auto rows = [&](size_t j0, size_t j1) {
    for (size_t j = j0; j < j1; j++) {
      dkgh::Zl x = dkgh::zl_from_u64(j + 1), y = dkgh::zl_from_u64(1);
      for (size_t e = L; e; e >>= 1) {
        if (e & 1) y = dkgh::zl_mul(y, x);
        x = dkgh::zl_mul(x, x);
      }
      dkgh::short_multipliers(y, (int)K, reinterpret_cast<uint8_t(*)[32]>(&mag[j * K * 32]), &sign[j * K]);
    }
  };
  const size_t nt = std::min<size_t>({(size_t)std::max(1u, std::thread::hardware_concurrency()), 16, (n + 63) / 64});
  std::vector<std::thread> th;
  for (size_t i = 1; i < nt; i++) th.emplace_back(rows, n * i / nt, n * (i + 1) / nt);
  rows(0, n / nt);
  for (auto& t : th) t.join();
}

void split_short(dkg_ctx* ctx, size_t n, size_t L, size_t K, const uint32_t** digits, const int16_t** top,
                 const uint32_t** scale) {
  uint32_t* dd = buf<uint32_t>(ctx, "v.sdig", 2 * 4 * 256 * n);
  int16_t* dt = buf<int16_t>(ctx, "v.stop", 2 * n);
  uint32_t* ds = buf<uint32_t>(ctx, "v.sscale", 32 * n);
  *digits = dd;
  *top = dt;
  *scale = ds;
  if (ctx->sdig_n == n && ctx->sdig_L == L && ctx->sdig_K == K) return;
  std::vector<uint8_t> mag;
  std::vector<int8_t> sign;
  short_vectors(n, L, K, mag, sign);
  std::vector<uint32_t> hd(2 * 256 * n, 0), hs(8 * n, 0);
  std::vector<int16_t> ht(n, -1);
  uint8_t r256[33] = {0};
  r256[32] = 1;
  const dkgh::Zl R = dkgh::zl_from_bytes_wide(r256, 33);
  for (size_t j = 0; j < n; j++) {
    for (size_t u = 0; u < K; u++) {
      int8_t d[256];
      int16_t tp;
      naf_digits(&mag[(j * K + u) * 32], d, &tp);
      ht[j] = std::max(ht[j], tp);
      for (int b = 0; b < 256; b++)
        hd[(u / 4) * 256 * n + 256 * j + b] |= (uint32_t)(uint8_t)(int8_t)(d[b] * sign[j * K + u]) << (8 * (u % 4));
    }
    const dkgh::Zl b = dkgh::zl_from_bytes_wide(&mag[j * K * 32], 32);
    uint8_t w[32];
    dkgh::zl_to_bytes(w, dkgh::zl_mul(b, R));
    memcpy(&hs[8 * j], w, 32);
  }
  h2d(ctx, dd, hd.data(), 4 * hd.size());
  h2d(ctx, dt, ht.data(), 2 * n);
  h2d(ctx, ds, hs.data(), 4 * hs.size());
  ctx->sdig_n = n;
  ctx->sdig_L = L;
  ctx->sdig_K = K;
}

void verify_device(dkg_ctx* ctx, size_t n, size_t t, const VerifySeg* segs, int nseg, bool timed,
                   const char* tag) {
  const size_t N = t + 1, D = segs[0].D;
  if (!D) return;
  if (nseg == 2 && (segs[1].D != D || segs[1].dealer_base != segs[0].dealer_base || segs[1].s != segs[0].s ||
                    segs[0].round != 2 || segs[1].round != 4)) {
    ctx->err = "verify_device: fused segments must be round 2 then round 4 of the same dealers";
    throw Fail{DKG_E_ARG};
  }
  const size_t groups = (D + 63) / 64, gw = 64 * nseg;
  const size_t npad = groups * gw;
  const size_t U = choose_split(ctx, npad, n, N), L = split_len(npad, n, N, U, ctx->combine_mode != 1), W = U * npad;
  const size_t Lr = last_piece_len(N, U, L);
  const bool whole = ctx->step_mode == 1 || ((ctx->step_mode == 0 || ctx->step_mode == 3) && stepping_whole_pays(npad, U, L, Lr));
  const bool step_ilp = use_ilp(ctx, false);
  ctx->last_split = (int)U;
  ctx->last_split_len = L;
  hipStream_t home = ctx->stream;
  uint8_t* pok = buf<uint8_t>(ctx, "v.pok", npad * N);
  uint8_t* dok = buf<uint8_t>(ctx, "v.dok", npad);
  uint32_t* Cpm = buf<uint32_t>(ctx, "v.Cpm", PTB * L * W);
  uint32_t* e0 = buf<uint32_t>(ctx, "v.binom0", PTB * L * W);
  uint32_t* e1 = buf<uint32_t>(ctx, "v.binom1", PTB * L * W);
  uint32_t* eT = buf<uint32_t>(ctx, "v.binomT", PTB * L * W);
  uint32_t* R = buf<uint32_t>(ctx, "v.R", PTB * W * n);
  uint32_t *sa = nullptr, *sb = nullptr;
  if (L > 512) {
    sa = buf<uint32_t>(ctx, "v.step_a", PTB * W * n);
    sb = buf<uint32_t>(ctx, "v.step_b", PTB * W * n);
  }
  const int8_t* ydig = nullptr;
  const int16_t* ytop = nullptr;
  const uint32_t *sdig = nullptr, *sscale = nullptr;
  const int16_t* stop = nullptr;
  const bool short_mult = U > 1 && U <= (ctx->addend_mode == 0 ? SHORT_MAX : 4) && ctx->combine_mode != 1;
  uint32_t* sflags = ctx->step_formula == 0
                         ? buf<uint32_t>(ctx, "v.sflags", 4 * dkgk::stepping_flag_words(npad, U)) : nullptr;
  ctx->last_step_flags = sflags;
  ctx->last_step_flag_words = sflags ? dkgk::stepping_flag_words(npad, U) : 0;
  uint32_t* Aff = short_mult && ctx->addend_mode == 0 ? buf<uint32_t>(ctx, "v.Aff", 4 * AFFP_WORDS_H * W * n) : nullptr;
  uint32_t* Rz = Aff ? buf<uint32_t>(ctx, "v.Rz", 40 * W * n) : nullptr;
  if (short_mult) split_short(ctx, n, L, U, &sdig, &stop, &sscale);
  else if (U > 1) split_digits(ctx, n, L, &ydig, &ytop);
  ctx->last_combine = U > 1 ? (short_mult ? 2 : 1) : 0;
  ctx->last_R = R;
  ctx->last_scale = sscale;
  ctx->last_dok = dok;
  if (npad != D * nseg || U * L != N) dkgk::fill_identity(L * W, Cpm, home);
  HCK(hipMemsetAsync(pok, 1, npad * N, home));
  const bool defer_r1 = ctx->r1_a && nseg == 2 && D == ctx->r1_D;
  for (int k = 0; k < nseg && !defer_r1; k++) {
    const uint32_t* ext = segs[k].round == 2 ? ctx->ext_E : ctx->ext_A;
    if (ext)
      dkgk::place_position_major(ext, ctx->ext_stride, D, N, W, Cpm, home, nseg, k, L, npad);
    else
      dkgk::decode_position_major(segs[k].Ccomp, D, N, W, Cpm, pok, home, nseg, k, L, npad);
  }
  dkgk::dealer_ok(npad, N, pok, dok, home);
  const bool defer_masks = ctx->shares_pending;
  for (int k = 0; k < nseg; k++)
    if (segs[k].extra_ok && !defer_masks) dkgk::and_dealer_mask(D, nseg, k, segs[k].extra_ok, dok, home);
  auto checks = [&](size_t d0, size_t d1, hipStream_t st, size_t j0 = 0, size_t jn = 0) {
    if (d1 <= d0 || !segs[0].dec) return;
    wait_shares(ctx, st);
    if (defer_masks)
      for (int k = 0; k < nseg; k++)
        if (segs[k].extra_ok) dkgk::and_dealer_mask(d1 - d0, nseg, k, segs[k].extra_ok + d0, dok + d0 * nseg, st);
    const VerifySeg& g = segs[0];
    if (nseg == 2) {
      uint32_t* acc = ctx->check_mode == 1 ? buf<uint32_t>(ctx, "v.acc", PTB * D * n) + d0 * n * PT_WORDS_H : nullptr;
      dkgk::check_both(d1 - d0, n, d0, g.dealer_base, g.self_mod ? g.self_mod : n, g.s, g.sp, R,
                       ctx->tab_gw, ctx->tab_hw, dok, g.dec, segs[1].dec, st, sscale, j0, jn, acc);
    } else {
      dkgk::check(d1 - d0, n, g.dealer_base + d0, 0, g.self_mod ? g.self_mod : n, g.round, g.s + d0 * n * 8,
                  g.round == 2 ? g.sp + d0 * n * 8 : nullptr, R + d0 * n * PT_WORDS_H, ctx->tab_gw, ctx->tab_hw,
                  dok + d0, g.dec + d0 * n, st, sscale);
    }
  };
  const bool saturating = (W / 64) * (L / 2) >= 4 * 1024;
  const bool long_stepping = (double)W * (double)L * (double)n >= 5e7 && npad >= 512;
  const size_t nsub = (saturating || long_stepping) ? std::min<size_t>(ctx->nsub, groups) : 1;
  const bool per_wave = ctx->binom_mode == 4 || ctx->binom_mode == 5 ||
                        (ctx->binom_mode == 0 && L > 1 && (double)npad / 64 * U >= DKG_BINOM_WAVE_GROUPS);
  ctx->last_binomial = per_wave ? 1 : 0;
  uint32_t* bflags = nullptr;
  const bool wave_ded = per_wave && DKG_BINOM_WAVE_DED && ctx->binom_mode != 5 &&
                        !(ctx->binom_mode == 0 && DKG_BINOM_WAVE_PF);
  const bool step_ded = !per_wave && ((DKG_BINOM_STEP_DED == 1 && ctx->binom_step_ded && ctx->binom_any) ||
                                      DKG_BINOM_STEP_DED == 2);
  if (ctx->step_formula == 0 && (wave_ded || (step_ded && DKG_BINOM_STEP_DED == 2))) {
    bflags = buf<uint32_t>(ctx, "v.bflags", 4 * (W / 64));
    HCK(hipMemsetAsync(bflags, 0, 4 * (W / 64), home));
  }
  uint32_t* bany = step_ded && DKG_BINOM_STEP_DED == 1 && ctx->step_formula == 0 ? ctx->binom_any : nullptr;
  const bool tails = ctx->step_mode != 3 && dkgk::stepping_tail_phases(L, n, U) > 1;
  uint32_t* tail_a = tails ? buf<uint32_t>(ctx, "v.tail_a", 4 * dkgk::stepping_tail_words(npad, L)) : nullptr;
  uint32_t* tail_b = tails ? buf<uint32_t>(ctx, "v.tail_b", 4 * dkgk::stepping_tail_words(npad, L)) : nullptr;
  auto chunk = [&](size_t g0, size_t g1, hipStream_t st, bool tm) {
    const size_t c0 = g0 * gw, w = (g1 - g0) * gw;
    if (defer_r1) {
      const size_t d0 = g0 * 64, d1 = std::min(D, g1 * 64);
      dkgk::commit_position_major(d1 - d0, N, ctx->r1_a + d0 * N * 8, ctx->r1_b + d0 * N * 8, ctx->tab_gw,
                                  ctx->tab_hw, Cpm + c0, W, L, npad, ctx->r1_A0 + d0, D, st);
    }
    if (tm) HCK(hipEventRecord(ctx->pev[0], st));
    const uint32_t* e;
    if (per_wave) {
      e = dkgk::binomial_wave(w, W, L, Cpm + c0, e0 + c0, st, U, npad, Lr,
                              DKG_BINOM_WAVE_COLMAJOR ? eT + c0 * L : nullptr,
                              ctx->binom_mode == 5 || (ctx->binom_mode == 0 && DKG_BINOM_WAVE_PF), bflags, c0, D,
                              (unsigned)gw);
    } else {
      dkgk::binom_init(w, W, L, Cpm + c0, e0 + c0, st, U, npad);
      uint32_t *bin = e0 + c0, *bout = e1 + c0;
      for (size_t r = 1; r < L; r++) {
        const double wps = (double)npad / 64 * U * (r + 1) / 1024;
        const bool ilp = use_ilp(ctx, wps < binom_ilp_waves());
        const bool pair = ctx->binom_mode == 2 || ((ctx->binom_mode == 0 || ctx->binom_mode == 3) &&
                                                   wps < DKG_BINOM_PAIR_WAVES);
        if (pair)
          (ilp ? dkgk_ilp::binom_step_pair : dkgk::binom_step_pair)(r, w, W, L, Cpm + c0, bin, bout, st, U, npad,
                                                                    Lr);
        else
          (ilp ? dkgk_ilp::binom_step : dkgk::binom_step)(r, w, W, L, Cpm + c0, bin, bout, st, U, npad, Lr,
                                                          bany ? bany : bflags, c0, D, (unsigned)gw, bany != nullptr,
                                                          binom_nt(r, npad * U), !ilp && wps < binom_il_waves());
        std::swap(bin, bout);
      }
      e = bin;
      if (bflags && DKG_BINOM_STEP_DED == 2)
        dkgk::binomial_wave_redo(w, W, L, Cpm + c0, bin, st, U, npad, Lr, bflags, c0, D, (unsigned)gw);
    }
    if (tm) HCK(hipEventRecord(ctx->pev[1], st));
    if (!per_wave || !DKG_BINOM_WAVE_COLMAJOR)
      dkgk::to_column_major(w, W, L, e, eT + c0 * L, U, npad, st);
    uint32_t* fl = sflags ? sflags + dkgk::stepping_flag_words(c0, U) : nullptr;
    if (fl) HCK(hipMemsetAsync(fl, 0, 4 * dkgk::stepping_flag_words(w, U), st));
    auto step = step_ilp ? dkgk_ilp::stepping : dkgk::stepping;
    if (!step(w, W, L, eT + c0 * L, n, R + c0 * n * PT_WORDS_H, sa ? sa + c0 * n * 40 : nullptr,
              sb ? sb + c0 * n * 40 : nullptr, st, U, npad, Lr, whole, fl, c0, D, (unsigned)gw,
              Rz ? Rz + c0 * n * 10 : nullptr, tail_a, tail_b))
      throw Fail{DKG_E_ARG};
    if (tm) HCK(hipEventRecord(ctx->pev[2], st));
    if (short_mult && Aff) {
      dkgk::affine_pieces(w, npad, U, n, R + c0 * n * PT_WORDS_H, Aff + c0 * n * AFFP_WORDS_H, st, Rz + c0 * n * 10);
      dkgk::combine_short_aff(w, npad, U, n, sdig, stop, Aff + c0 * n * AFFP_WORDS_H, R + c0 * n * PT_WORDS_H, st);
    } else if (short_mult) dkgk::combine_short(w, npad, U, n, sdig, stop, R + c0 * n * PT_WORDS_H, st);
    else dkgk::combine(w, npad, U, n, ydig, ytop, R + c0 * n * PT_WORDS_H, st);
    if (tm) HCK(hipEventRecord(ctx->pev[3], st));
    checks(g0 * 64, std::min(D, g1 * 64), st);
    if (tm) HCK(hipEventRecord(ctx->pev[4], st));
  };
  ctx->timed_tag.clear();
  if (nsub <= 1) {
    chunk(0, groups, home, timed);
    if (timed) ctx->timed_tag = tag;
  } else {
    HCK(hipEventRecord(ctx->fork, home));
    size_t g0 = 0;
    for (size_t c = 0; c < nsub; c++) {
      const size_t g1 = groups * (c + 1) / nsub;
      HCK(hipStreamWaitEvent(ctx->sub[c], ctx->fork, 0));
      chunk(g0, g1, ctx->sub[c], false);
      HCK(hipEventRecord(ctx->join[c], ctx->sub[c]));
      HCK(hipStreamWaitEvent(home, ctx->join[c], 0));
      g0 = g1;
    }
  }
  check_launch(ctx);
}

void verify_one(dkg_ctx* ctx, size_t n, size_t t, int round, size_t D, size_t dealer_base, const uint32_t* Ccomp,
                const uint32_t* s, const uint32_t* sp, uint8_t* dec, bool timed, const uint8_t* extra_ok = nullptr) {
  VerifySeg g{round, D, dealer_base, Ccomp, s, sp, dec, extra_ok};
  verify_device(ctx, n, t, &g, 1, timed, round == 2 ? "r2" : "r4");
}

template <typename F>
void verify_rounds_group(dkg_ctx* ctx, size_t n, size_t t, size_t D, size_t dealer_base, const uint32_t* Ecomp,
                         const uint32_t* Acomp, const uint32_t* s, const uint32_t* sp, uint8_t* dec2, uint8_t* dec4,
                         hipEvent_t after2, F&& between, const uint8_t* e_ok, const uint8_t* a_ok,
                         bool host_between) {
  if (ctx->overlap) {
    VerifySeg g[2] = {{2, D, dealer_base, Ecomp, s, sp, dec2, e_ok}, {4, D, dealer_base, Acomp, s, nullptr, dec4, a_ok}};
    verify_device(ctx, n, t, g, 2, true, "r24");
    if (after2) HCK(hipEventRecord(after2, ctx->stream));
    if (host_between) {
      sync(ctx);
      collect_phases(ctx);
    }
    between();
  } else {
    VerifySeg g2{2, D, dealer_base, Ecomp, s, sp, dec2, e_ok};
    verify_device(ctx, n, t, &g2, 1, true, "r2");
    if (after2) HCK(hipEventRecord(after2, ctx->stream));
    sync(ctx);
    collect_phases(ctx);
    between();
    verify_one(ctx, n, t, 4, D, dealer_base, Acomp, s, nullptr, dec4, true, a_ok);
    sync(ctx);
    collect_phases(ctx);
  }
}

const uint32_t* vinv_table(dkg_ctx* ctx, size_t N) {
  uint32_t* dev = buf<uint32_t>(ctx, "v.vinv", 4 * 11 * N * N);
  if (ctx->vinv_N == N) return dev;
  using dkgh::Zl;
  const Zl zero = dkgh::zl_from_u64(0);
  std::vector<Zl> M(N + 1, zero);
  M[0] = dkgh::zl_from_u64(1);
  for (size_t m = 0; m < N; m++) {
    const Zl xm = dkgh::zl_from_u64(m + 1);
    for (size_t k = m + 1; k > 0; k--) M[k] = dkgh::zl_sub(M[k - 1], dkgh::zl_mul(xm, M[k]));
    M[0] = dkgh::zl_sub(zero, dkgh::zl_mul(xm, M[0]));
  }
  uint8_t r256[33] = {0};
  r256[32] = 1;
  const Zl R = dkgh::zl_from_bytes_wide(r256, 33);
  std::vector<uint32_t> host(11 * N * N);
  std::vector<Zl> q(N);
  for (size_t j = 0; j < N; j++) {
    const Zl xj = dkgh::zl_from_u64(j + 1);
    q[N - 1] = M[N];
    for (size_t k = N - 1; k > 0; k--) q[k - 1] = dkgh::zl_add(M[k], dkgh::zl_mul(xj, q[k]));
    Zl den = zero;
    for (size_t k = N; k-- > 0;) den = dkgh::zl_add(dkgh::zl_mul(den, xj), q[k]);
    const Zl scale = dkgh::zl_mul(dkgh::zl_inv(den), R);
    for (size_t k = 0; k < N; k++) {
      uint8_t b[33] = {0};
      dkgh::zl_to_bytes(b, dkgh::zl_mul(q[k], scale));
      for (size_t a = 0; a < 11; a++) {
        const size_t by = 3 * a;
        host[(j * 11 + a) * N + k] = (uint32_t)b[by] | (uint32_t)b[by + 1] << 8 | (uint32_t)b[by + 2] << 16;
      }
    }
  }
  h2d(ctx, dev, host.data(), 4 * host.size());
  ctx->vinv_N = N;
  return dev;
}

template <typename F>
void verify_rounds_interp(dkg_ctx* ctx, size_t n, size_t t, size_t D, size_t dealer_base, const uint32_t* Ecomp,
                          const uint32_t* Acomp, const uint32_t* s, const uint32_t* sp, uint8_t* dec2, uint8_t* dec4,
                          hipEvent_t after2, F&& between, const uint8_t* e_ok, const uint8_t* a_ok) {
  const size_t N = t + 1;
  hipStream_t st = ctx->stream;
  if (D) {
    HCK(hipEventRecord(ctx->pev[0], st));
    const uint32_t *Ee, *Ae;
    size_t cs;
    uint8_t* dokE = buf<uint8_t>(ctx, "i.dokE", D);
    uint8_t* dokA = buf<uint8_t>(ctx, "i.dokA", D);
    if (ctx->ext_E) {
      Ee = ctx->ext_E;
      Ae = ctx->ext_A;
      cs = ctx->ext_stride;
      HCK(hipMemsetAsync(dokE, 1, D, st));
      HCK(hipMemsetAsync(dokA, 1, D, st));
    } else {
      uint32_t* ee = buf<uint32_t>(ctx, "i.Eext", PTB * D * N);
      uint32_t* ae = buf<uint32_t>(ctx, "i.Aext", PTB * D * N);
      uint8_t* pok = buf<uint8_t>(ctx, "i.pok", D * N);
      dkgk::decode_points(Ecomp, D * N, ee, D * N, pok, st);
      dkgk::dealer_ok(D, N, pok, dokE, st);
      dkgk::decode_points(Acomp, D * N, ae, D * N, pok, st);
      dkgk::dealer_ok(D, N, pok, dokA, st);
      Ee = ee;
      Ae = ae;
      cs = D * N;
    }
    dkgk::and_mask(D, e_ok, dokE, st);
    dkgk::and_mask(D, a_ok, dokA, st);
    const uint32_t* WT = vinv_table(ctx, N);
    uint32_t* Fa = buf<uint32_t>(ctx, "i.F", 32 * D * N);
    uint32_t* Fb = buf<uint32_t>(ctx, "i.Fp", 32 * D * N);
    dkgk::interp(D, N, n, WT, s, sp, Fa, Fb, st);
    HCK(hipEventRecord(ctx->pev[1], st));
    uint8_t* okE = buf<uint8_t>(ctx, "i.okE", D * N);
    uint8_t* okA = buf<uint8_t>(ctx, "i.okA", D * N);
    dkgk::coef_check(D, N, Fa, Fb, Ee, Ae, cs, ctx->tab_gw, ctx->tab_hw, okE, okA, st);
    uint8_t* cE = buf<uint8_t>(ctx, "i.cE", D);
    uint8_t* cA = buf<uint8_t>(ctx, "i.cA", D);
    dkgk::dealer_ok(D, N, okE, cE, st);
    dkgk::dealer_ok(D, N, okA, cA, st);
    HCK(hipEventRecord(ctx->pev[2], st));
    dkgk::interp_decide(D, n, N, dealer_base, n, s, sp, Fa, Fb, dokE, dokA, cE, cA, ctx->tab_gw, ctx->tab_hw, dec2,
                        dec4, st);
    HCK(hipEventRecord(ctx->pev[3], st));
    check_launch(ctx);
    std::vector<uint8_t> h_dE(D), h_dA(D), h_cE(D), h_cA(D);
    d2h(ctx, h_dE.data(), dokE, D);
    d2h(ctx, h_dA.data(), dokA, D);
    d2h(ctx, h_cE.data(), cE, D);
    d2h(ctx, h_cA.data(), cA, D);
    sync(ctx);
// ... 1236 lines not shown
    if (!sclk_mhz || !busy_ms || !iters) return DKG_E_ARG;
    int cus = 0, wall_khz = 0;
    HCK(hipDeviceGetAttribute(&cus, hipDeviceAttributeMultiprocessorCount, ctx->device));
    HCK(hipDeviceGetAttribute(&wall_khz, hipDeviceAttributeWallClockRate, ctx->device));
    if (cus <= 0 || wall_khz <= 0) return DKG_E_DEVICE;
    const size_t waves = (size_t)cus * 16;
    unsigned long long* d = buf<unsigned long long>(ctx, "clock_probe", 2 * 8 * waves);
    hipLaunchKernelGGL(k_clock_probe, dim3((unsigned)(waves / 4)), dim3(256), 0, ctx->stream, iters, d);
    check_launch(ctx);
    std::vector<unsigned long long> h(2 * waves);
    d2h(ctx, h.data(), d, 2 * 8 * waves);
    sync(ctx);
    std::vector<double> mhz(waves), ms(waves);
    for (size_t w = 0; w < waves; w++) {
      const double real_us = (double)h[2 * w + 1] / wall_khz * 1e3;
      mhz[w] = real_us > 0 ? (double)h[2 * w] / real_us : 0.0;
      ms[w] = real_us / 1e3;
    }
    std::nth_element(mhz.begin(), mhz.begin() + waves / 2, mhz.end());
    std::nth_element(ms.begin(), ms.begin() + waves / 2, ms.end());
    *sclk_mhz = mhz[waves / 2];
    *busy_ms = ms[waves / 2];
    return DKG_OK;
  });
}

int dkg_ctx_create(int device, dkg_ctx** out) {
  if (!out) return DKG_E_ARG;
  *out = nullptr;
  dkg_ctx* ctx = new dkg_ctx();
  ctx->device = device;
  int rc = guarded(ctx, [&] {
    int least = 0, greatest = 0;
    HCK(hipDeviceGetStreamPriorityRange(&least, &greatest));
    HCK(hipStreamCreateWithPriority(&ctx->stream, hipStreamNonBlocking, greatest));
    for (auto& e : ctx->ev) HCK(hipEventCreate(&e));
    for (auto& e : ctx->pev) HCK(hipEventCreate(&e));
    for (auto& e : ctx->hev) HCK(hipEventCreate(&e));
    for (auto& st : ctx->sub) HCK(hipStreamCreateWithPriority(&st, hipStreamNonBlocking, greatest));
    HCK(hipStreamCreateWithPriority(&ctx->side, hipStreamNonBlocking, least));
    HCK(hipEventCreateWithFlags(&ctx->side_fork, hipEventDisableTiming));
    HCK(hipEventCreateWithFlags(&ctx->shares_done, hipEventDisableTiming));
    HCK(hipEventCreateWithFlags(&ctx->pub_done, hipEventDisableTiming));
    HCK(hipEventCreateWithFlags(&ctx->terms_done, hipEventDisableTiming));
    HCK(hipEventCreateWithFlags(&ctx->fork, hipEventDisableTiming));
    for (auto& e : ctx->join) HCK(hipEventCreateWithFlags(&e, hipEventDisableTiming));
    HCK(hipMalloc(&ctx->tab_g, COMB_BYTES));
    HCK(hipMalloc(&ctx->tab_h, COMB_BYTES));
    HCK(hipMalloc(&ctx->tab_gw, COMBW_BYTES));
    HCK(hipMalloc(&ctx->tab_hw, COMBW_BYTES));
    bool ok = false;
    comb_for_point(ctx, BASEPOINT, ctx->tab_g, &ok, ctx->tab_gw);
    if (!ok) {
      ctx->err = "basepoint failed to decode on device";
      return DKG_E_DEVICE;
    }
    return DKG_OK;
  });
  if (rc != DKG_OK) {
    fprintf(stderr, "dkg_ctx_create: %s\n", ctx->err.c_str());
    dkg_ctx_destroy(ctx);
    return rc;
  }
  *out = ctx;
  return DKG_OK;
}

void dkg_ctx_destroy(dkg_ctx* ctx) {
  if (!ctx) return;
  (void)hipSetDevice(ctx->device);
  if (ctx->stream) (void)hipDeviceSynchronize();
  for (auto& kv : ctx->bufs) (void)hipFree(kv.second.first);
  for (auto& kv : ctx->hbufs) (void)hipHostFree(kv.second.first);
  if (ctx->tab_g) (void)hipFree(ctx->tab_g);
  if (ctx->tab_h) (void)hipFree(ctx->tab_h);
  if (ctx->tab_gw) (void)hipFree(ctx->tab_gw);
  if (ctx->tab_hw) (void)hipFree(ctx->tab_hw);
  for (auto& e : ctx->ev)
    if (e) (void)hipEventDestroy(e);
  for (auto& e : ctx->pev)
    if (e) (void)hipEventDestroy(e);
  for (auto& e : ctx->hev)
    if (e) (void)hipEventDestroy(e);
  for (auto& e : ctx->join)
    if (e) (void)hipEventDestroy(e);
  for (auto& e : ctx->bf_pool)
    if (e) (void)hipEventDestroy(e);
  if (ctx->fork) (void)hipEventDestroy(ctx->fork);
  for (auto& st : ctx->sub)
    if (st) (void)hipStreamDestroy(st);
  if (ctx->stream) (void)hipStreamDestroy(ctx->stream);
  if (ctx->side) (void)hipStreamDestroy(ctx->side);
  if (ctx->side_fork) (void)hipEventDestroy(ctx->side_fork);
  if (ctx->shares_done) (void)hipEventDestroy(ctx->shares_done);
  if (ctx->pub_done) (void)hipEventDestroy(ctx->pub_done);
  delete ctx;
}

const char* dkg_ctx_last_error(const dkg_ctx* ctx) { return ctx ? ctx->err.c_str() : "null context"; }

double dkg_ctx_phase_ms(const dkg_ctx* ctx, const char* name) {
  if (!ctx || !name) return -1.0;
  auto it = ctx->phase_ms.find(name);
  return it == ctx->phase_ms.end() ? -1.0 : it->second;
}

int dkg_ctx_set_streams(dkg_ctx* ctx, int nsub) {
  if (!ctx || nsub < 1 || nsub > dkg_ctx::MAX_SUB) return DKG_E_ARG;
  ctx->nsub = nsub;
  return DKG_OK;
}

int dkg_ctx_set_verify_mode(dkg_ctx* ctx, int mode) {
  if (!ctx || mode < 0 || mode > 1) return DKG_E_ARG;
  ctx->verify_mode = mode;
  return DKG_OK;
}

size_t dkg_ctx_fallback_rows(const dkg_ctx* ctx) { return ctx ? ctx->fallback_rows : 0; }

int dkg_ctx_set_split(dkg_ctx* ctx, int pieces) {
  if (!ctx || pieces < 0 || pieces > 16) return DKG_E_ARG;
  ctx->split = pieces;
  return DKG_OK;
}

int dkg_ctx_set_binomial(dkg_ctx* ctx, int mode) {
  if (!ctx || mode < 0 || mode > 5) return DKG_E_ARG;
  ctx->binom_mode = mode;
  return DKG_OK;
}

int dkg_ctx_set_check(dkg_ctx* ctx, int mode) {
  if (!ctx || mode < 0 || mode > 1) return DKG_E_ARG;
  ctx->check_mode = mode;
  return DKG_OK;
}

int dkg_ctx_set_field_mode(dkg_ctx* ctx, int mode) {
  if (!ctx || mode < 0 || mode > 2) return DKG_E_ARG;
  ctx->fe_mode = mode;
  return DKG_OK;
}

int dkg_ctx_set_stepping(dkg_ctx* ctx, int mode) {
  if (!ctx || mode < 0 || mode > 3) return DKG_E_ARG;
  ctx->step_mode = mode;
  return DKG_OK;
}

int dkg_ctx_last_split(const dkg_ctx* ctx) { return ctx ? ctx->last_split : 0; }
size_t dkg_ctx_last_split_len(const dkg_ctx* ctx) { return ctx ? ctx->last_split_len : 0; }
int dkg_ctx_set_combine(dkg_ctx* ctx, int mode) {
  if (!ctx || mode < 0 || mode > 2) return DKG_E_ARG;
  ctx->combine_mode = mode;
  return DKG_OK;
}
int dkg_ctx_last_combine(const dkg_ctx* ctx) { return ctx ? ctx->last_combine : 0; }
int dkg_ctx_last_binomial(const dkg_ctx* ctx) { return ctx ? ctx->last_binomial : 0; }
int dkg_ctx_set_stepping_formula(dkg_ctx* ctx, int mode) {
  if (!ctx || mode < 0 || mode > 1) return DKG_E_ARG;
  ctx->step_formula = mode;
  return DKG_OK;
}
long long dkg_ctx_stepping_redos(dkg_ctx* ctx) {
  if (!ctx) return -1;
  if (!ctx->last_step_flags) return 0;
  try {
    std::vector<uint32_t> h(ctx->last_step_flag_words);
    sync(ctx);
    HCK(hipMemcpy(h.data(), ctx->last_step_flags, 4 * h.size(), hipMemcpyDeviceToHost));
    long long c = 0;
    for (uint32_t x : h) c += x != 0;
    return c;
  } catch (const Fail& f) {
    return -1;
  }
}
int dkg_ctx_binomial_reruns(dkg_ctx* ctx) { return ctx ? ctx->last_binom_rerun : -1; }
int dkg_ctx_set_addends(dkg_ctx* ctx, int mode) {
  if (!ctx || mode < 0 || mode > 1) return DKG_E_ARG;
  ctx->addend_mode = mode;
  return DKG_OK;
}
int dkg_split_multipliers(size_t n, size_t L, int pieces, uint8_t* mag, int8_t* sign) {
  if (!n || !L || pieces < 2 || pieces > (int)SHORT_MAX || !mag || !sign) return DKG_E_ARG;
  try {
    std::vector<uint8_t> m;
    std::vector<int8_t> sg;
    short_vectors(n, L, (size_t)pieces, m, sg);
    memcpy(mag, m.data(), m.size());
    memcpy(sign, sg.data(), sg.size());
  } catch (const std::exception&) {
    return DKG_E_NOMEM;
  }
  return DKG_OK;
}

double dkg_split_model_ms(size_t columns, size_t n, size_t t, int pieces) {
  if (pieces < 1 || t + 1 < (size_t)pieces) return -1;
  return split_model_ms(columns, n, t + 1, (size_t)pieces);
}

size_t dkg_split_len(size_t columns, size_t n, size_t t, int pieces) {
  if (pieces < 1 || t + 1 < (size_t)pieces) return 0;
  return split_len(columns, n, t + 1, (size_t)pieces);
}

int dkg_ctx_set_overlap(dkg_ctx* ctx, int on) {
  if (!ctx) return DKG_E_ARG;
  ctx->overlap = on != 0;
  return DKG_OK;
}

int dkg_env_check(size_t threshold, size_t nr_members) {
  if (nr_members == 0 || !(threshold < (nr_members + 1) / 2)) return DKG_E_ARG;
  return DKG_OK;
}

int dkg_env_init(dkg_ctx* ctx, size_t threshold, size_t nr_members, const uint8_t* ck, size_t ck_len,
                 uint8_t h_out[32]) {
  int rc = dkg_env_check(threshold, nr_members);
  if (rc != DKG_OK) {
    if (ctx) ctx->err = "threshold must be < (nr_members + 1) / 2 (committee.rs:73)";
    return rc;
  }
  return guarded(ctx, [&] {
    uint8_t hash[64];
    dkgh::blake2b(hash, 64, ck, ck_len);
    uint32_t* in = buf<uint32_t>(ctx, "h_in", 64);
    uint32_t* ext = buf<uint32_t>(ctx, "h_ext", PTB);
    uint32_t* comp = buf<uint32_t>(ctx, "h_comp", 32);
    h2d(ctx, in, hash, 64);
    dkgk::from_uniform(in, ext, ctx->stream);
    dkgk::encode_points(ext, 1, 1, comp, ctx->stream);
    check_launch(ctx);
    d2h(ctx, ctx->h, comp, 32);
    sync(ctx);
    bool ok = false;
    comb_for_point(ctx, ctx->h, ctx->tab_h, &ok, ctx->tab_hw);
    if (!ok) return DKG_E_DEVICE;
    ctx->have_h = true;
    ctx->threshold = threshold;
    ctx->nr_members = nr_members;
    if (h_out) memcpy(h_out, ctx->h, 32);
    return DKG_OK;
  });
}

int dkg_msm_batch(dkg_ctx* ctx, size_t B, size_t N, const uint8_t* scalars, const uint8_t* points, uint8_t* out) {
  return guarded(ctx, [&] {
    if (B == 0) return DKG_OK;
    uint32_t* sc = upload_scalars(ctx, "msm_sc", scalars, B * N);
    uint32_t* pc = buf<uint32_t>(ctx, "msm_pc", 32 * B * N);
    uint32_t* pe = buf<uint32_t>(ctx, "msm_pe", PTB * B * N);
    uint8_t* ok = buf<uint8_t>(ctx, "msm_ok", B * N);
    h2d(ctx, pc, points, 32 * B * N);
    dkgk::decode_points(pc, B * N, pe, B * N, ok, ctx->stream);
    uint32_t* oe = buf<uint32_t>(ctx, "msm_oe", PTB * B);
    uint32_t* oc = buf<uint32_t>(ctx, "msm_oc", 32 * B);
    uint32_t* mt = buf<uint32_t>(ctx, "msm_tab", 4 * 15 * PT_WORDS_H * B * N);
  dkgk::msm_batch(B, N, sc, pe, B * N, mt, oe, ctx->stream);
    dkgk::encode_points(oe, B, B, oc, ctx->stream);
    check_launch(ctx);
    std::vector<uint8_t> okh(B * N);
    d2h(ctx, okh.data(), ok, B * N);
    d2h(ctx, out, oc, 32 * B);
    sync(ctx);
    for (auto v : okh)
      if (!v) {
        ctx->err = "msm: a point failed to decode";
        return DKG_E_DECODE;
      }
    return DKG_OK;
  });
}

int dkg_fixed_base_batch(dkg_ctx* ctx, const uint8_t base[32], size_t count, const uint8_t* scalars, uint8_t* out) {
  return guarded(ctx, [&] {
    if (count == 0) return DKG_OK;
    const uint32_t* tab = ctx->tab_gw;
    if (base && memcmp(base, BASEPOINT, 32) == 0) {
      base = nullptr;
    } else if (base && ctx->have_h && ctx->tab_hw && memcmp(base, ctx->h, 32) == 0) {
      tab = ctx->tab_hw;
      base = nullptr;
    }
    if (base) {
      uint32_t* t = buf<uint32_t>(ctx, "fb_tabw", COMBW_BYTES);
      if (!ctx->fb_valid || memcmp(ctx->fb_base, base, 32) != 0) {
        ctx->fb_valid = false;
        bool ok = false;
        comb_for_point(ctx, base, nullptr, &ok, t);
        if (!ok) {
          ctx->err = "fixed_base: base point failed to decode";
          return DKG_E_DECODE;
        }
        memcpy(ctx->fb_base, base, 32);
        ctx->fb_valid = true;
      }
      tab = t;
    }
    uint32_t* sc = upload_scalars(ctx, "fb_sc", scalars, count);
    uint32_t* oe = buf<uint32_t>(ctx, "fb_oe", PTB * count);
    uint32_t* oc = buf<uint32_t>(ctx, "fb_oc", 32 * count);
    dkgk::fixed_base(count, sc, tab, oe, ctx->stream);
    dkgk::encode_points(oe, count, count, oc, ctx->stream);
    check_launch(ctx);
    d2h(ctx, out, oc, 32 * count);
    sync(ctx);
    return DKG_OK;
  });
}

int dkg_poly_eval_batch(dkg_ctx* ctx, size_t D, size_t N, const uint8_t* coeffs, size_t M, const uint32_t* xs,
                        uint8_t* out) {
  return guarded(ctx, [&] {
    if (D == 0 || M == 0) return DKG_OK;
    if (N == 0) return DKG_E_ARG;
    for (size_t m = 0; m < M; m++)
      if (xs[m] >= (1u << 24)) {
        ctx->err = "poly_eval: evaluation points must be < 2^24";
        return DKG_E_ARG;
      }
    uint32_t* c = upload_scalars(ctx, "pe_c", coeffs, D * N);
    uint32_t* x = buf<uint32_t>(ctx, "pe_x", 4 * M);
    uint32_t* o = buf<uint32_t>(ctx, "pe_o", 32 * D * M);
    h2d(ctx, x, xs, 4 * M);
    dkgk::poly_eval(D, N, c, M, x, o, ctx->stream);
    check_launch(ctx);
    d2h(ctx, out, o, 32 * D * M);
    sync(ctx);
    return DKG_OK;
  });
}

int dkg_points_valid_batch(dkg_ctx* ctx, size_t count, const uint8_t* points, uint8_t* ok) {
  return guarded(ctx, [&] {
    if (count == 0) return DKG_OK;
    uint32_t* pc = buf<uint32_t>(ctx, "pv_c", 32 * count);
    uint32_t* pe = buf<uint32_t>(ctx, "pv_e", PTB * count);
    uint8_t* od = buf<uint8_t>(ctx, "pv_ok", count);
    h2d(ctx, pc, points, 32 * count);
    dkgk::decode_points(pc, count, pe, count, od, ctx->stream);
    check_launch(ctx);
// ... 1377 lines not shown
```

include/dkg_amd.h:

```cpp
#ifndef DKG_AMD_H
#define DKG_AMD_H
#include <stddef.h>
#include <stdint.h>

#ifdef __cplusplus
extern "C" {
#endif

#define DKG_OK 0
#define DKG_E_ARG (-1)
#define DKG_E_DECODE (-2)
#define DKG_E_DEVICE (-3)
#define DKG_E_NOMEM (-4)

#define DKG_REJECT 0
#define DKG_ACCEPT 1
#define DKG_SELF 2
#define DKG_SKIPPED 3
#define DKG_MISSING 4

typedef struct dkg_ctx dkg_ctx;

int dkg_ctx_create(int device, dkg_ctx **out);
void dkg_ctx_destroy(dkg_ctx *ctx);
const char *dkg_ctx_last_error(const dkg_ctx *ctx);
double dkg_ctx_phase_ms(const dkg_ctx *ctx, const char *name);
int dkg_ctx_set_streams(dkg_ctx *ctx, int nsub);
int dkg_ctx_set_overlap(dkg_ctx *ctx, int on);
int dkg_ctx_set_split(dkg_ctx *ctx, int pieces);
int dkg_ctx_set_stepping(dkg_ctx *ctx, int mode);
int dkg_ctx_set_field_mode(dkg_ctx *ctx, int mode);
int dkg_ctx_set_binomial(dkg_ctx *ctx, int mode);
int dkg_ctx_set_check(dkg_ctx *ctx, int mode);
int dkg_ctx_set_verify_mode(dkg_ctx *ctx, int mode);
size_t dkg_ctx_fallback_rows(const dkg_ctx *ctx);
int dkg_ctx_last_split(const dkg_ctx *ctx);
size_t dkg_ctx_last_split_len(const dkg_ctx *ctx);
double dkg_split_model_ms(size_t columns, size_t n, size_t t, int pieces);
size_t dkg_split_len(size_t columns, size_t n, size_t t, int pieces);
int dkg_ctx_set_combine(dkg_ctx *ctx, int mode);
int dkg_ctx_last_combine(const dkg_ctx *ctx);
int dkg_ctx_last_binomial(const dkg_ctx *ctx);
int dkg_ctx_set_addends(dkg_ctx *ctx, int mode);
int dkg_ctx_set_stepping_formula(dkg_ctx *ctx, int mode);
long long dkg_ctx_stepping_redos(dkg_ctx *ctx);
int dkg_ctx_binomial_reruns(dkg_ctx *ctx);
int dkg_split_multipliers(size_t n, size_t L, int pieces, uint8_t *mag, int8_t *sign);
int dkg_device_count(void);
int dkg_ctx_clock_probe(dkg_ctx *ctx, unsigned iters, double *sclk_mhz, double *busy_ms);
int dkg_device_pci_bus_id(int device, char *buf, int len);

int dkg_env_init(dkg_ctx *ctx, size_t threshold, size_t nr_members, const uint8_t *ck_bytes, size_t ck_len,
                 uint8_t h_out[32]);
int dkg_env_check(size_t threshold, size_t nr_members);

int dkg_msm_batch(dkg_ctx *ctx, size_t B, size_t N, const uint8_t *scalars, const uint8_t *points, uint8_t *out);
int dkg_fixed_base_batch(dkg_ctx *ctx, const uint8_t base[32], size_t count, const uint8_t *scalars, uint8_t *out);
int dkg_poly_eval_batch(dkg_ctx *ctx, size_t D, size_t N, const uint8_t *coeffs, size_t M, const uint32_t *xs,
                        uint8_t *out);
int dkg_points_valid_batch(dkg_ctx *ctx, size_t count, const uint8_t *points, uint8_t *ok);

int dkg_share_gen(dkg_ctx *ctx, size_t D, size_t n, size_t t, const uint8_t *a, const uint8_t *b, uint8_t *E,
                  uint8_t *A, uint8_t *s, uint8_t *s_prime);
int dkg_share_gen_device(dkg_ctx *ctx, size_t D, size_t n, size_t t, const void *d_a, const void *d_b, void *d_E,
                         void *d_A, void *d_s, void *d_s_prime);

int dkg_verify_pairs(dkg_ctx *ctx, size_t n, size_t t, int round, size_t d0, size_t d1, const uint8_t *C,
                     const uint8_t *s, const uint8_t *s_prime, uint8_t *decision);
int dkg_verify_receiver(dkg_ctx *ctx, size_t n, size_t t, int round, size_t j, const uint8_t *C, const uint8_t *s,
                        const uint8_t *s_prime, uint8_t *decision);

typedef struct {
  uint8_t *E, *A;
  uint8_t *s, *s_prime;
  uint8_t *dec2, *dec4;
  uint8_t *qualified;
  uint8_t *r2_error;
  uint8_t *r4_error;
  int32_t *complaints2;
  uint8_t *reconstruct;
  uint8_t *final_share;
  uint8_t *public_share;
  uint8_t mpk[32];
  int32_t n_qualified;
  int32_t phase4_error;
  double ms_round1, ms_round2, ms_round3, ms_round4, ms_finalise, ms_total;
} dkg_ceremony_out;

int dkg_ceremony_run(dkg_ctx *ctx, size_t n, size_t t, const uint8_t *a, const uint8_t *b, dkg_ceremony_out *out);
int dkg_ceremony_verify(dkg_ctx *ctx, size_t n, size_t t, const uint8_t *E, const uint8_t *A, const uint8_t *s,
                        const uint8_t *s_prime, dkg_ceremony_out *out);
int dkg_ceremony_verify_fetched(dkg_ctx *ctx, size_t n, size_t t, const uint8_t *E, const uint8_t *A,
                                const uint8_t *s, const uint8_t *s_prime, const uint8_t *fetched1,
                                const uint8_t *fetched3, dkg_ceremony_out *out);
int dkg_ceremony_run_device(dkg_ctx *ctx, size_t n, size_t t, const void *d_a, const void *d_b,
                            dkg_ceremony_out *out);
int dkg_ceremony_shard_device(dkg_ctx *ctx, size_t n, size_t t, size_t d0, size_t d1, const void *d_a,
                              const void *d_b, void *d_dec2, void *d_dec4, void *d_A0, void *d_partial,
                              double *ms_total);
int dkg_ceremony_shard_verify_device(dkg_ctx *ctx, size_t n, size_t t, size_t d0, size_t d1, const void *d_E,
                                     const void *d_A, const void *d_s, const void *d_s_prime, void *d_dec2,
                                     void *d_dec4, void *d_A0, void *d_partial, double *ms_total);
int dkg_ceremony_shard_recon_device(dkg_ctx *ctx, size_t n, size_t t, size_t d0, size_t d1, const uint8_t *qualified,
                                    const uint8_t *reconstruct, const uint8_t *r2_error, const uint8_t *r4_error,
                                    const void *d_s, void *d_terms, int32_t *recovery_error);
int dkg_scalar_sum_device(dkg_ctx *ctx, size_t rows, size_t n, const void *d_in, const void *d_mask, void *d_out);
int dkg_point_sum_device(dkg_ctx *ctx, size_t count, const void *d_points, const void *d_mask, void *d_out);

void dkg_shard_range(size_t n, size_t world_size, size_t rank, size_t *d0, size_t *d1);
size_t dkg_shard_rows(size_t n, size_t world_size);

typedef struct {
  uint8_t *qualified;
  int32_t *complaints2;
  uint8_t *r2_error;
  uint8_t *reconstruct;
  uint8_t *r4_error;
  int32_t n_qualified;
  int32_t phase4_error;
} dkg_shard_outcome;

int dkg_shard_combine_device(dkg_ctx *ctx, size_t n, size_t t, size_t world_size, const void *d_dec2_g,
                             const void *d_dec4_g, void *d_dec2, void *d_dec4, dkg_shard_outcome *out);
size_t dkg_packed_row_words(size_t n);
int dkg_fixed_base_windows(void);
int dkg_key_comb_windows(void);
int dkg_decisions_pack_device(dkg_ctx *ctx, size_t rows, size_t nvalid, size_t n, size_t d0, const void *d_dec,
                              void *d_packed);
int dkg_shard_combine_packed_device(dkg_ctx *ctx, size_t n, size_t t, size_t world_size, const void *d_pack2_g,
                                    const void *d_pack4_g, void *d_dec2, void *d_dec4, dkg_shard_outcome *out);
int dkg_shard_finalise_device(dkg_ctx *ctx, size_t n, size_t t, size_t world_size, const void *d_terms_g,
                              const void *d_partials_g, const uint8_t *qualified, int phase4_error,
                              void *d_final_share, void *d_public_share, uint8_t *mpk);

typedef struct dkg_multi dkg_multi;
int dkg_multi_create(const int *devices, int ndev, dkg_multi **out);
void dkg_multi_destroy(dkg_multi *m);
int dkg_multi_size(const dkg_multi *m);
dkg_ctx *dkg_multi_ctx(dkg_multi *m, int shard);
const char *dkg_multi_last_error(const dkg_multi *m);
double dkg_multi_phase_ms(const dkg_multi *m, const char *name);
int dkg_multi_env_init(dkg_multi *m, size_t threshold, size_t nr_members, const uint8_t *ck_bytes, size_t ck_len,
                       uint8_t h_out[32]);
int dkg_multi_ceremony_run(dkg_multi *m, size_t n, size_t t, const uint8_t *a, const uint8_t *b,
                           dkg_ceremony_out *out);
int dkg_multi_ceremony_run_device(dkg_multi *m, size_t n, size_t t, const void *const *d_a, const void *const *d_b,
                                  dkg_ceremony_out *out);
int dkg_multi_ceremony_verify(dkg_multi *m, size_t n, size_t t, const uint8_t *E, const uint8_t *A, const uint8_t *s,
                              const uint8_t *s_prime, dkg_ceremony_out *out);

#define DKG_FIN_OK 0
#define DKG_FIN_R2_ERROR 1
#define DKG_FIN_R4_ERROR 2
#define DKG_FIN_PHASE4_ERROR 3
#define DKG_FIN_INSUFFICIENT 4
#define DKG_FIN_PANIC 5
int dkg_finalise_parties(dkg_ctx *ctx, size_t n, size_t t, const uint8_t *qualified, const uint8_t *reconstruct,
                         const uint8_t *r2_error, const uint8_t *r4_error, const uint8_t *disclosed, const uint8_t *A0,
                         const uint8_t *s, uint8_t *mpk, int32_t *status, int32_t *recovery_index);

typedef struct {
  uint8_t *mpk;
  int32_t *n_qualified;
  uint8_t *phase4_error;
  uint8_t *qualified;
  uint8_t *r2_error;
  uint8_t *r4_error;
  int32_t *complaints2;
  uint8_t *reconstruct;
  uint8_t *final_share;
  uint8_t *public_share;
  uint8_t *dec2, *dec4;
  double ms_round1, ms_checks, ms_round3, ms_finalise, ms_total;
} dkg_batch_out;

int dkg_ceremony_batch_device(dkg_ctx *ctx, size_t B, size_t n, size_t t, const void *d_a, const void *d_b,
                              dkg_batch_out *out);
int dkg_ceremony_batch_verify(dkg_ctx *ctx, size_t B, size_t n, size_t t, const uint8_t *E, const uint8_t *A,
                              const uint8_t *s, const uint8_t *s_prime, dkg_batch_out *out);

int dkg_member_keys(dkg_ctx *ctx, const uint8_t master[32], uint32_t ceremony, size_t n, uint8_t *sk, uint8_t *pk);
int dkg_enc_randomness(const uint8_t master[32], uint32_t ceremony, size_t d0, size_t D, size_t n, size_t t,
                       uint8_t *r);
int dkg_enc_randomness_device(dkg_ctx *ctx, const uint8_t master[32], uint32_t ceremony0, size_t B, size_t d0,
                              size_t D, size_t n, size_t t, void *d_r);
int dkg_encrypt_shares(dkg_ctx *ctx, size_t D, size_t n, const uint8_t *pk, const uint8_t *s, const uint8_t *s_prime,
                       const uint8_t *r, uint8_t *e1, uint8_t *ct);
int dkg_decrypt_shares(dkg_ctx *ctx, size_t D, size_t n, const uint8_t *sk, const uint8_t *e1, const uint8_t *ct,
                       uint8_t *s, uint8_t *s_prime, uint8_t *ok);
int dkg_ceremony_run_full_device(dkg_ctx *ctx, size_t n, size_t t, const void *d_a, const void *d_b, const void *d_r,
                                 const uint8_t *sk, const uint8_t *pk, dkg_ceremony_out *out);
int dkg_ceremony_verify_full(dkg_ctx *ctx, size_t n, size_t t, const uint8_t *E, const uint8_t *A, const uint8_t *e1,
                             const uint8_t *ct, const uint8_t *sk, dkg_ceremony_out *out);

int dkg_member_keys_batch(dkg_ctx *ctx, const uint8_t master[32], uint32_t ceremony0, size_t B, size_t n, uint8_t *sk,
                          uint8_t *pk);
int dkg_encrypt_shares_batch(dkg_ctx *ctx, size_t B, size_t n, const uint8_t *pk, const uint8_t *s,
                             const uint8_t *s_prime, const uint8_t *r, uint8_t *e1, uint8_t *ct);
int dkg_decrypt_shares_batch(dkg_ctx *ctx, size_t B, size_t n, const uint8_t *sk, const uint8_t *e1, const uint8_t *ct,
                             uint8_t *s, uint8_t *s_prime, uint8_t *ok);
// ... 57 lines not shown
```

Baseline: 13.15 million verified shares/s.

## Recombine split pieces with joint sparse form digits over precomputed pair sums

Replaces the per-piece NAF recombination with Shamir-style joint sparse form recoding of piece pairs. A new kernel precomputes P0+P1 and P0-P1 for each pair, and a new combine kernel streams those affine sums through wave-uniform event lists, so one addition covers positions where both digits are nonzero. The lattice search for short multipliers also scores candidates by JSF cost. This aims to cut the number of additions in the recombination step, at the price of extra memory for the pair-sum planes, an extra kernel pass and more host-side digit preprocessing.

```diff
diff --git a/dkg_amd/_lib.py b/dkg_amd/_lib.py
--- a/dkg_amd/_lib.py
+++ b/dkg_amd/_lib.py
@@ -107,6 +107,8 @@
     L.dkg_ctx_clock_probe.argtypes = [p, ctypes.c_uint, ctypes.POINTER(ctypes.c_double), ctypes.POINTER(ctypes.c_double)]
     L.dkg_device_pci_bus_id.argtypes = [ctypes.c_int, ctypes.c_char_p, ctypes.c_int]
     L.dkg_split_multipliers.argtypes = [sz, sz, ctypes.c_int, p, p]
+    L.dkg_jsf_digits.argtypes = [p, p, p, p, p]
+    L.dkg_split_digits.argtypes = [sz, sz, ctypes.c_int, ctypes.c_int, p, p]
     L.dkg_ctx_phase_ms.argtypes = [p, ctypes.c_char_p]
     L.dkg_ctx_phase_ms.restype = ctypes.c_double
     L.dkg_env_check.argtypes = [sz, sz]
@@ -199,7 +201,7 @@
     "dkg_env_check", "dkg_msm_batch", "dkg_fixed_base_batch", "dkg_poly_eval_batch",
     "dkg_points_valid_batch", "dkg_share_gen", "dkg_verify_pairs", "dkg_verify_receiver",
     "dkg_ctx_set_split", "dkg_ctx_set_stepping", "dkg_ctx_set_field_mode", "dkg_ctx_set_binomial", "dkg_ctx_set_check", "dkg_ctx_last_split", "dkg_ctx_last_split_len", "dkg_ctx_set_verify_mode", "dkg_ctx_fallback_rows", "dkg_split_model_ms", "dkg_split_len",
-    "dkg_ctx_set_combine", "dkg_ctx_last_combine", "dkg_ctx_last_binomial", "dkg_ctx_set_addends", "dkg_ctx_set_stepping_formula", "dkg_ctx_stepping_redos", "dkg_ctx_binomial_reruns", "dkg_split_multipliers",
+    "dkg_ctx_set_combine", "dkg_ctx_last_combine", "dkg_ctx_last_binomial", "dkg_ctx_set_addends", "dkg_ctx_set_stepping_formula", "dkg_ctx_stepping_redos", "dkg_ctx_binomial_reruns", "dkg_split_multipliers", "dkg_jsf_digits", "dkg_split_digits",
     "dkg_ctx_clock_probe", "dkg_device_pci_bus_id",
     "dkg_ceremony_run", "dkg_ceremony_verify", "dkg_ceremony_verify_fetched", "dkg_ceremony_run_device", "dkg_ceremony_shard_device",
     "dkg_ceremony_shard_verify_device",
diff --git a/dkg_amd/csrc/ge25519.h b/dkg_amd/csrc/ge25519.h
--- a/dkg_amd/csrc/ge25519.h
+++ b/dkg_amd/csrc/ge25519.h
@@ -326,6 +326,44 @@
     qa.v[i] = neg ? q.ypx.v[i] : q.ymx.v[i];
     qb.v[i] = neg ? q.ymx.v[i] : q.ypx.v[i];
   }
+  if constexpr (IL && DKG_PW) {
+    fe u;
+    fe_sub(t, p.Y, p.X);
+    fe_add(u, p.Y, p.X);
+    fe_mul2(a, t, qa, b, u, qb);
+  } else {
+    fe_sub(t, p.Y, p.X);
+    fe_mul(a, t, qa);
+    fe_add(t, p.Y, p.X);
+    fe_mul(b, t, qb);
+  }
+  fe_sub(e, b, a);
+  fe_add(h, b, a);
+  fe_mul(a, p.T, q.xy2d);
+  fe na;
+  fe_neg(na, a);
+  fe_cmov(a, na, neg);
+  fe_dbl(b, p.Z);
+  fe_carry(b, b);
+  fe_sub(t, b, a);
+  fe_add(b, b, a);
+  if constexpr (IL && DKG_PW) {
+    fe_mul2(r.X, e, t, r.Y, b, h);
+    if (with_t) fe_mul2(r.Z, b, t, r.T, e, h);
+    else fe_mul(r.Z, b, t);
+  } else {
+    fe_mul(r.X, e, t);
+    fe_mul(r.Y, b, h);
+    fe_mul(r.Z, b, t);
+    if (with_t) fe_mul(r.T, e, h);
+  }
+}
+
+template <bool IL = false>
+DKG_DEV void ge_madd_swapped(ge_p3& r, const ge_p3& p, const ge_aff& q, bool neg, bool with_t = true) {
+  fe a, b, e, h, t;
+  const fe& qa = q.ymx;
+  const fe& qb = q.ypx;
   if constexpr (IL && DKG_PW) {
     fe u;
     fe_sub(t, p.Y, p.X);
diff --git a/dkg_amd/csrc/host_crypto.h b/dkg_amd/csrc/host_crypto.h
--- a/dkg_amd/csrc/host_crypto.h
+++ b/dkg_amd/csrc/host_crypto.h
@@ -21,6 +21,8 @@
 Zl zl_inv(const Zl& a);
 bool zl_is_zero(const Zl& a);
 
-bool short_multipliers(const Zl& y, int K, uint8_t (*mag)[32], int8_t* sign);
+bool short_multipliers(const Zl& y, int K, uint8_t (*mag)[32], int8_t* sign, bool jsf = false);
+bool jsf_digits(const uint8_t a[32], const uint8_t b[32], int8_t* da, int8_t* db, int16_t* top,
+                int npos = 256);
 
 }
diff --git a/dkg_amd/csrc/kernels.hip b/dkg_amd/csrc/kernels.hip
--- a/dkg_amd/csrc/kernels.hip
+++ b/dkg_amd/csrc/kernels.hip
@@ -1495,6 +1495,174 @@
     hipLaunchKernelGGL((k_combine_aff<5, 2>), grid, dim3(64), 0, stream, width, pstride, nrecv, digits, top, A, R, j0);
 }
 
+__global__ __launch_bounds__(256) void k_pair_sums(size_t width, size_t pstride, size_t pieces, size_t nrecv,
+                                                   uint32_t* R, uint32_t* Rz, size_t j0, size_t jn) {
+  const size_t gid = (size_t)blockIdx.x * blockDim.x + threadIdx.x;
+  const size_t j = j0 + gid % jn, rest = gid / jn, c = rest % width, p = rest / width;
+  if (p >= pieces / 2) return;
+  const size_t e0 = ((2 * p) * pstride + c) * nrecv + j, e1 = e0 + pstride * nrecv;
+  const size_t es = ((pieces + 2 * p) * pstride + c) * nrecv + j, ed = es + pstride * nrecv;
+  ge_p3 a, s;
+  ge_cached q;
+  {
+    ge_p3 b;
+    pt_load_aos(b, R, e1);
+    ge_to_cached(q, b);
+  }
+  pt_load_aos(a, R, e0);
+  fe ym, yp, f, g, x, y, e, h;
+  fe_mul(x, a.T, q.T2d);
+  fe_mul(y, a.Z, q.Z2);
+  fe_sub(f, y, x);
+  fe_add(g, y, x);
+  fe_sub(ym, a.Y, a.X);
+  fe_add(yp, a.Y, a.X);
+  fe_mul(s.Z, g, f);
+  fe_mul(x, ym, q.YmX);
+  fe_mul(y, yp, q.YpX);
+  fe_sub(e, y, x);
+  fe_add(h, y, x);
+  fe_mul(s.X, e, f);
+  fe_mul(s.Y, g, h);
+  fe_mul(s.T, e, h);
+  pt_store_aos<DKG_STEP_NT != 0>(R, es, s);
+  fe_mul(x, ym, q.YpX);
+  fe_mul(y, yp, q.YmX);
+  fe_sub(e, y, x);
+  fe_add(h, y, x);
+  fe_mul(s.X, e, g);
+  fe_mul(s.Y, f, h);
+  fe_mul(s.T, e, h);
+  pt_store_aos<DKG_STEP_NT != 0>(R, ed, s);
+  uint2* zs = reinterpret_cast<uint2*>(Rz + es * 10);
+  uint2* zd = reinterpret_cast<uint2*>(Rz + ed * 10);
+#pragma unroll
+  for (int k = 0; k < 5; k++) zs[k] = zd[k] = make_uint2(s.Z.v[2 * k], s.Z.v[2 * k + 1]);
+}
+
+void pair_sums(size_t width, size_t pstride, size_t pieces, size_t nrecv, uint32_t* R, uint32_t* Rz,
+               hipStream_t stream, size_t j0, size_t jn) {
+  if (!jn) jn = nrecv - j0;
+  if (!width || !jn || pieces < 2) return;
+  const size_t lanes = (pieces / 2) * width * jn;
+  hipLaunchKernelGGL(k_pair_sums, dim3((unsigned)((lanes + 255) / 256)), dim3(256), 0, stream, width, pstride, pieces,
+                     nrecv, R, Rz, j0, jn);
+}
+
+DKG_DEV void jsf_fetch(ge_aff& q, const uint32_t* __restrict__ A0, uint32_t slot, size_t plane, uint32_t e) {
+  if (e == JSF_EV_NONE) return;
+  asm volatile("" : "+v"(slot));
+  const uint32_t* a = A0 + (size_t)slot * AFFP_WORDS + (e & 3u) * plane;
+  const uint2* f0 = reinterpret_cast<const uint2*>(a + ((e & 4u) ? 10 : 0));
+  const uint2* f1 = reinterpret_cast<const uint2*>(a + ((e & 4u) ? 0 : 10));
+  const uint2* f2 = reinterpret_cast<const uint2*>(a + 20);
+#pragma unroll
+  for (int i = 0; i < 5; i++) {
+    const uint2 u = f0[i], v = f1[i], w = f2[i];
+    q.ypx.v[2 * i] = u.x;
+    q.ypx.v[2 * i + 1] = u.y;
+    q.ymx.v[2 * i] = v.x;
+    q.ymx.v[2 * i + 1] = v.y;
+    q.xy2d.v[2 * i] = w.x;
+    q.xy2d.v[2 * i + 1] = w.y;
+  }
+}
+
+struct JsfStream {
+  ge_aff q;
+  const uint32_t* A0;
+  uint32_t slot;
+  size_t plane;
+  const uint32_t* ev;
+  uint32_t next;
+  int k;
+};
+
+template <int P, int K, int KL>
+DKG_DEV void jsf_position(ge_p3& acc, uint32_t w, const uint32_t* qs, const ge_aff* qr, JsfStream& s, bool last) {
+  if constexpr (2 * P < K) {
+    const int e0 = (int8_t)(w >> (16 * P)), e1 = (int8_t)(w >> (16 * P + 8));
+    bool t = last;
+    if constexpr (2 * P + 2 < K) t = t || (w >> (16 * P + 16)) != 0;
+    if (e0 != 0 && e1 != 0) {
+      ge_madd_swapped<DKG_AFF_IL != 0>(acc, acc, s.q, e0 < 0, t);
+      const uint32_t e = s.next;
+      s.next = (uint32_t)__builtin_amdgcn_readfirstlane(s.ev[s.k]);
+      s.k++;
+      jsf_fetch(s.q, s.A0, s.slot, s.plane, e);
+    } else if (e0 != 0 || e1 != 0) {
+      constexpr int U0 = 2 * P, U1 = 2 * P + 1;
+      if constexpr (U1 < KL) {
+        const int u = e0 != 0 ? U0 : U1;
+        ge_madd_lds<DKG_AFF_IL != 0>(acc, acc, qs + u * AFF_WORDS * 64 + threadIdx.x, (e0 | e1) < 0, 64, t);
+      } else if (e0 != 0) {
+        if constexpr (U0 < KL) ge_madd_lds<DKG_AFF_IL != 0>(acc, acc, qs + U0 * AFF_WORDS * 64 + threadIdx.x, e0 < 0, 64, t);
+        else ge_madd_signed<DKG_AFF_IL != 0>(acc, acc, qr[U0 - KL], e0 < 0, t);
+      } else {
+        ge_madd_signed<DKG_AFF_IL != 0>(acc, acc, qr[U1 - KL], e1 < 0, t);
+      }
+    }
+    jsf_position<P + 1, K, KL>(acc, w, qs, qr, s, last);
+  }
+}
+
+template <int K, int KL>
+__global__ __launch_bounds__(64, 2) void k_combine_jsf(size_t width, size_t pstride, size_t nrecv,
+                                                       const uint32_t* __restrict__ digits,
+                                                       const int16_t* __restrict__ top,
+                                                       const uint32_t* __restrict__ ev,
+                                                       const uint32_t* __restrict__ A, uint32_t* __restrict__ R,
+                                                       size_t j0) {
+  static_assert(K % 2 == 0 && K <= 4, "whole pairs in one digit word");
+  __shared__ uint32_t qs[KL * AFF_WORDS * 64];
+  const size_t c = (size_t)blockIdx.x * 64 + threadIdx.x;
+  const size_t j = j0 + blockIdx.y;
+  const bool live = c < width;
+  const size_t cc = live ? c : 0;
+  ge_aff qr[K - KL > 0 ? K - KL : 1];
+  aff_addends<0, K, KL>(qs, qr, A, pstride, cc, nrecv, j);
+  const uint32_t* dw = digits + j * 256;
+  const int tp = top[j];
+  JsfStream s;
+  s.A0 = A + ((size_t)K * pstride * nrecv + j) * AFFP_WORDS;
+  s.slot = (uint32_t)(cc * nrecv);
+  s.plane = pstride * nrecv * AFFP_WORDS;
+  s.ev = ev + j * JSF_EV_WORDS;
+  s.next = (uint32_t)__builtin_amdgcn_readfirstlane(s.ev[1]);
+  s.k = 2;
+#pragma unroll
+  for (int u = 0; u < K - KL; u++) {
+#pragma unroll
+    for (int i = 0; i < 10; i++)
+      asm volatile("" : "+v"(qr[u].ypx.v[i]), "+v"(qr[u].ymx.v[i]), "+v"(qr[u].xy2d.v[i]));
+  }
+  fe_zero(s.q.ypx);
+  fe_zero(s.q.ymx);
+  fe_zero(s.q.xy2d);
+  jsf_fetch(s.q, s.A0, s.slot, s.plane, (uint32_t)__builtin_amdgcn_readfirstlane(s.ev[0]));
+  ge_p3 acc;
+  ge_identity(acc);
+#pragma unroll 1
+  for (int b = tp; b >= 0; b--) {
+    const uint32_t w = (uint32_t)__builtin_amdgcn_readfirstlane(dw[b]);
+    if (b != tp) ge_dbl_lean<DKG_AFF_IL != 0>(acc, acc, w != 0 || b == 0);
+    jsf_position<0, K, KL>(acc, w, qs, qr, s, b == 0);
+  }
+  if (live) pt_store_aos<DKG_COMB_NT != 0>(R, (size_t)s.slot + j, acc);
+}
+
+void combine_short_jsf(size_t width, size_t pstride, size_t pieces, size_t nrecv, const uint32_t* digits,
+                       const int16_t* top, const uint32_t* ev, const uint32_t* A, uint32_t* R, hipStream_t stream,
+                       size_t j0, size_t jn) {
+  if (!jn) jn = nrecv - j0;
+  if (!width || !jn || (pieces != 2 && pieces != 4)) return;
+  const dim3 grid((unsigned)((width + 63) / 64), (unsigned)jn);
+  if (pieces == 2)
+    hipLaunchKernelGGL((k_combine_jsf<2, 1>), grid, dim3(64), 0, stream, width, pstride, nrecv, digits, top, ev, A, R, j0);
+  else
+    hipLaunchKernelGGL((k_combine_jsf<4, 2>), grid, dim3(64), 0, stream, width, pstride, nrecv, digits, top, ev, A, R, j0);
+}
+
 void combine(size_t width, size_t pstride, size_t pieces, size_t nrecv, const int8_t* digits, const int16_t* top,
              uint32_t* R, hipStream_t stream) {
   if (!width || !nrecv || pieces < 2) return;
diff --git a/dkg_amd/csrc/kernels_decl.inc b/dkg_amd/csrc/kernels_decl.inc
--- a/dkg_amd/csrc/kernels_decl.inc
+++ b/dkg_amd/csrc/kernels_decl.inc
@@ -73,6 +73,13 @@
 void combine_short_aff(size_t width, size_t pstride, size_t pieces, size_t nrecv, const uint32_t* digits,
                        const int16_t* top, const uint32_t* A, uint32_t* R, hipStream_t stream, size_t j0 = 0,
                        size_t jn = 0);
+void pair_sums(size_t width, size_t pstride, size_t pieces, size_t nrecv, uint32_t* R, uint32_t* Rz,
+               hipStream_t stream, size_t j0 = 0, size_t jn = 0);
+constexpr uint32_t JSF_EV_NONE = 0xffu;
+constexpr size_t JSF_EV_WORDS = 384;
+void combine_short_jsf(size_t width, size_t pstride, size_t pieces, size_t nrecv, const uint32_t* digits,
+                       const int16_t* top, const uint32_t* ev, const uint32_t* A, uint32_t* R, hipStream_t stream,
+                       size_t j0 = 0, size_t jn = 0);
 void check(size_t ndealers, size_t nrecv, size_t dealer_base, size_t recv_base, size_t nmod, int round,
            const uint32_t* s, const uint32_t* sp, const uint32_t* R, const uint32_t* tab_g,
            const uint32_t* tab_h, const uint8_t* dealer_ok, uint8_t* decision, hipStream_t stream,
diff --git a/dkg_amd/csrc/lattice.cpp b/dkg_amd/csrc/lattice.cpp
--- a/dkg_amd/csrc/lattice.cpp
+++ b/dkg_amd/csrc/lattice.cpp
@@ -97,11 +97,31 @@
     if (h) len = 64 * i + 64 - __builtin_clzll(h);
   }
 }
-double chain_cost(const I512* v, int K) {
+void i_jsf_shape(const I512& a, const I512& b, int& len, int& weight) {
+  const I512 ma = i_neg_p(a) ? i_neg(a) : a, mb = i_neg_p(b) ? i_neg(b) : b;
+  uint8_t ba[32], bb[32];
+  for (int i = 0; i < 32; i++) {
+    ba[i] = (uint8_t)(ma.w[i / 8] >> (8 * (i % 8)));
+    bb[i] = (uint8_t)(mb.w[i / 8] >> (8 * (i % 8)));
+  }
+  int8_t da[256], db[256];
+  int16_t tp;
+  const int bits = i_bits(ma) > i_bits(mb) ? i_bits(ma) : i_bits(mb);
+  jsf_digits(ba, bb, da, db, &tp, bits + 2 < 256 ? bits + 2 : 256);
+  len = tp + 1;
+  weight = 0;
+  for (int i = 0; i <= tp; i++) weight += (da[i] | db[i]) != 0;
+}
+double chain_cost(const I512* v, int K, bool jsf) {
   int top = 0, adds = 0;
   for (int u = 0; u < K; u++) {
     int len, w;
-    i_naf_shape(v[u], len, w);
+    if (jsf && u + 1 < K) {
+      i_jsf_shape(v[u], v[u + 1], len, w);
+      u++;
+    } else {
+      i_naf_shape(v[u], len, w);
+    }
     top = top > len ? top : len;
     adds += w;
   }
@@ -159,7 +179,40 @@
 
 }
 
-bool short_multipliers(const Zl& y, int K, uint8_t (*mag)[32], int8_t* sign) {
+bool jsf_digits(const uint8_t a[32], const uint8_t b[32], int8_t* da, int8_t* db, int16_t* top, int npos) {
+  uint64_t k[2][5] = {{0}};
+  for (int i = 0; i < 32; i++) {
+    k[0][i / 8] |= (uint64_t)a[i] << (8 * (i % 8));
+    k[1][i / 8] |= (uint64_t)b[i] << (8 * (i % 8));
+  }
+  int c[2] = {0, 0};
+  *top = -1;
+  for (int i = 0; i < npos; i++) {
+    int l[2], u[2];
+    for (int s = 0; s < 2; s++) {
+      const int w = i >> 6, sh = i & 63;
+      uint64_t lo = k[s][w] >> sh;
+      if (sh > 61) lo |= k[s][w + 1] << (64 - sh);
+      l[s] = (int)(lo & 7) + c[s];
+    }
+    for (int s = 0; s < 2; s++) {
+      if (!(l[s] & 1)) {
+        u[s] = 0;
+      } else {
+        u[s] = (l[s] & 3) == 1 ? 1 : -1;
+        if (((l[s] & 7) == 3 || (l[s] & 7) == 5) && (l[1 - s] & 3) == 2) u[s] = -u[s];
+      }
+    }
+    for (int s = 0; s < 2; s++)
+      if (2 * c[s] == 1 + u[s]) c[s] = 1 - c[s];
+    da[i] = (int8_t)u[0];
+    db[i] = (int8_t)u[1];
+    if (u[0] | u[1]) *top = (int16_t)i;
+  }
+  return c[0] == 0 && c[1] == 0;
+}
+
+bool short_multipliers(const Zl& y, int K, uint8_t (*mag)[32], int8_t* sign, bool jsf) {
   if (K < 2 || K > KMAX) return false;
   I512 B[KMAX][KMAX];
   Zl p = zl_from_u64(1), pw[KMAX];
@@ -210,7 +263,7 @@
       for (int u = 0; u < K; u++) mult[i][c + CR][u] = i_mul_shift(B[i][u], c, 0);
   I512 v[KMAX];
   for (int u = 0; u < K; u++) v[u] = i_from_zl(pw[u]);
-  double best = chain_cost(v, K);
+  double best = chain_cost(v, K, jsf);
   I512 win[KMAX];
   bool have = false;
   int ncomb = 1;
@@ -231,7 +284,7 @@
       small = i_bits(c[u]) < 253;
     }
     if (!small) continue;
-    const double cost = chain_cost(c, K);
+    const double cost = chain_cost(c, K, jsf);
     if (!(cost < best)) continue;
     if (zl_is_zero(zl_of(c[0]))) continue;
     best = cost;
diff --git a/dkg_amd/csrc/runtime.hip b/dkg_amd/csrc/runtime.hip
--- a/dkg_amd/csrc/runtime.hip
+++ b/dkg_amd/csrc/runtime.hip
@@ -67,6 +67,7 @@
   int last_binom_rerun = 0;
   int addend_mode = 0;
   size_t sdig_n = 0, sdig_L = 0, sdig_K = 0;
+  int sdig_jsf = -1;
   const uint32_t* last_R = nullptr;
   const uint32_t* last_scale = nullptr;
   const uint8_t* last_dok = nullptr;
@@ -300,7 +301,10 @@
 #define DKG_AUTO_SHORT5 0
 #endif
 
-double split_model_ms(size_t cols, size_t n, size_t N, size_t U, size_t L, bool short_mult) {
+constexpr int SM_POWERS = 0, SM_NAF = 1, SM_JSF = 2;
+bool jsf_built(size_t U) { return U == 2 || U == 4; }
+
+double split_model_ms(size_t cols, size_t n, size_t N, size_t U, size_t L, int short_mult) {
   const double DBL = 1000, ADD = 1400, SIMDS = 1024, THR = 4.5, LAT = 8, LAT_ILP = 6, LAUNCH = 3e-3 * 2.4e6;
   const size_t Lr = last_piece_len(N, U, L), off = L - Lr;
   auto cost = [&](size_t m) {
@@ -337,7 +341,9 @@
   }
   if (U > 1) {
     const double bits = 253.0 * (U - 1) / U;
-    const double per = short_mult && U <= SHORT_MAX ? bits * 950 + U * bits / 3 * ADD
+    const bool jsf = short_mult == SM_JSF && jsf_built(U);
+    const double adds = jsf ? (U / 2) * bits / 2 + (U % 2) * bits / 3 : U * bits / 3;
+    const double per = short_mult && U <= SHORT_MAX ? bits * 950 + adds * ADD + (jsf ? 2 * (U / 2) * 23.0 / 8 * ADD : 0.0)
                                             : (U % 2 == 0 ? 253 * 950 + 85 * ADD : 0.0) +
                                                   ((U + 1) / 2 - 1) * (253 * 950 + 170 * ADD);
     const double waves = (double)cols / 64 * n;
@@ -347,7 +353,7 @@
   return cyc / 2.4e6;
 }
 
-size_t split_len(size_t cols, size_t n, size_t N, size_t U, bool short_mult = true) {
+size_t split_len(size_t cols, size_t n, size_t N, size_t U, int short_mult = SM_JSF) {
   const size_t L1 = (N + U - 1) / U;
   if (U == 1) return L1;
   const size_t L64 = (L1 + 63) / 64 * 64;
@@ -355,20 +361,25 @@
   return split_model_ms(cols, n, N, U, L64, short_mult) < split_model_ms(cols, n, N, U, L1, short_mult) ? L64 : L1;
 }
 
-double split_model_ms(size_t cols, size_t n, size_t N, size_t U, bool short_mult = true) {
+double split_model_ms(size_t cols, size_t n, size_t N, size_t U, int short_mult = SM_JSF) {
   return split_model_ms(cols, n, N, U, split_len(cols, n, N, U, short_mult), short_mult);
+}
+
+int short_kind(const dkg_ctx* ctx) {
+  if (ctx->combine_mode == 1) return SM_POWERS;
+  return ctx->combine_mode == 3 || ctx->addend_mode != 0 ? SM_NAF : SM_JSF;
 }
 
 size_t choose_split(dkg_ctx* ctx, size_t cols, size_t n, size_t N) {
   if (ctx->split > 0) return std::min<size_t>((size_t)ctx->split, N);
-  const bool sm = ctx->combine_mode != 1;
+  const int sm = short_kind(ctx);
   const double base = split_model_ms(cols, n, N, 1, sm);
   std::vector<double> ms(17, 0.0);
   double best_ms = base;
   size_t umax = 1;
   for (size_t U = 2; U <= 16; U++) {
     if (N < 64 * U) break;
-    ms[U] = split_model_ms(cols, n, N, U, sm && (U <= 4 || (ctx->addend_mode == 0 && DKG_AUTO_SHORT5)));
+    ms[U] = split_model_ms(cols, n, N, U, U <= 4 || (ctx->addend_mode == 0 && DKG_AUTO_SHORT5) ? sm : SM_POWERS);
     best_ms = std::min(best_ms, ms[U]);
     umax = U;
   }
@@ -429,7 +440,7 @@
   ctx->ydig_L = L;
 }
 
-void short_vectors(size_t n, size_t L, size_t K, std::vector<uint8_t>& mag, std::vector<int8_t>& sign) {
+void short_vectors(size_t n, size_t L, size_t K, std::vector<uint8_t>& mag, std::vector<int8_t>& sign, bool jsf) {
   mag.assign(n * K * 32, 0);
   sign.assign(n * K, 1);
   auto rows = [&](size_t j0, size_t j1) {
@@ -439,7 +450,7 @@
         if (e & 1) y = dkgh::zl_mul(y, x);
         x = dkgh::zl_mul(x, x);
       }
-      dkgh::short_multipliers(y, (int)K, reinterpret_cast<uint8_t(*)[32]>(&mag[j * K * 32]), &sign[j * K]);
+      dkgh::short_multipliers(y, (int)K, reinterpret_cast<uint8_t(*)[32]>(&mag[j * K * 32]), &sign[j * K], jsf);
     }
   };
   const size_t nt = std::min<size_t>({(size_t)std::max(1u, std::thread::hardware_concurrency()), 16, (n + 63) / 64});
@@ -449,43 +460,84 @@
   for (auto& t : th) t.join();
 }
 
-void split_short(dkg_ctx* ctx, size_t n, size_t L, size_t K, const uint32_t** digits, const int16_t** top,
-                 const uint32_t** scale) {
+bool short_digit_words(size_t n, size_t K, bool jsf, const std::vector<uint8_t>& mag, const std::vector<int8_t>& sign,
+                       std::vector<uint32_t>& hd, std::vector<int16_t>& ht, std::vector<uint32_t>* hev) {
+  hd.assign(2 * 256 * n, 0);
+  ht.assign(n, -1);
+  if (hev) hev->assign(dkgk::JSF_EV_WORDS * n, dkgk::JSF_EV_NONE);
+  for (size_t j = 0; j < n; j++) {
+    auto put = [&](size_t u, const int8_t* d) {
+      for (int b = 0; b < 256; b++)
+        hd[(u / 4) * 256 * n + 256 * j + b] |= (uint32_t)(uint8_t)(int8_t)(d[b] * sign[j * K + u]) << (8 * (u % 4));
+    };
+    for (size_t u = 0; u < K; u++) {
+      int8_t d[256], d1[256];
+      int16_t tp;
+      if (jsf && u + 1 < K) {
+        if (!dkgh::jsf_digits(&mag[(j * K + u) * 32], &mag[(j * K + u + 1) * 32], d, d1, &tp)) return false;
+        put(u, d);
+        put(u + 1, d1);
+        u++;
+      } else {
+        naf_digits(&mag[(j * K + u) * 32], d, &tp);
+        put(u, d);
+      }
+      ht[j] = std::max(ht[j], tp);
+    }
+    if (jsf && hev) {
+      size_t k = 0;
+      for (int b = ht[j]; b >= 0; b--) {
+        const uint32_t w = hd[256 * j + b];
+        for (size_t p = 0; p < K / 2 && p < 2; p++) {
+          const int e0 = (int8_t)(w >> (16 * p)), e1 = (int8_t)(w >> (16 * p + 8));
+          if (!e0 || !e1) continue;
+          if (k + 2 >= dkgk::JSF_EV_WORDS) return false;
+          (*hev)[dkgk::JSF_EV_WORDS * j + k++] = (uint32_t)(2 * p + (e0 != e1) + (e0 < 0 ? 4 : 0));
+        }
+      }
+    }
+  }
+  return true;
+}
+
+void split_short(dkg_ctx* ctx, size_t n, size_t L, size_t K, bool jsf, const uint32_t** digits, const int16_t** top,
+                 const uint32_t** scale, const uint32_t** events) {
   uint32_t* dd = buf<uint32_t>(ctx, "v.sdig", 2 * 4 * 256 * n);
   int16_t* dt = buf<int16_t>(ctx, "v.stop", 2 * n);
   uint32_t* ds = buf<uint32_t>(ctx, "v.sscale", 32 * n);
+  uint32_t* de = buf<uint32_t>(ctx, "v.sev", 4 * dkgk::JSF_EV_WORDS * n);
   *digits = dd;
   *top = dt;
   *scale = ds;
-  if (ctx->sdig_n == n && ctx->sdig_L == L && ctx->sdig_K == K) return;
+  *events = de;
+  if (ctx->sdig_n == n && ctx->sdig_L == L && ctx->sdig_K == K && ctx->sdig_jsf == (int)jsf) return;
   std::vector<uint8_t> mag;
   std::vector<int8_t> sign;
-  short_vectors(n, L, K, mag, sign);
-  std::vector<uint32_t> hd(2 * 256 * n, 0), hs(8 * n, 0);
-  std::vector<int16_t> ht(n, -1);
+  short_vectors(n, L, K, mag, sign, jsf);
+  std::vector<uint32_t> hd, hs(8 * n, 0), hev;
+  std::vector<int16_t> ht;
+  if (!short_digit_words(n, K, jsf, mag, sign, hd, ht, &hev)) {
+    ctx->err = "split_short: a joint sparse form does not fit its digit words";
+    throw Fail{DKG_E_ARG};
+  }
   uint8_t r256[33] = {0};
   r256[32] = 1;
   const dkgh::Zl R = dkgh::zl_from_bytes_wide(r256, 33);
   for (size_t j = 0; j < n; j++) {
-    for (size_t u = 0; u < K; u++) {
-      int8_t d[256];
-      int16_t tp;
-      naf_digits(&mag[(j * K + u) * 32], d, &tp);
-      ht[j] = std::max(ht[j], tp);
-      for (int b = 0; b < 256; b++)
-        hd[(u / 4) * 256 * n + 256 * j + b] |= (uint32_t)(uint8_t)(int8_t)(d[b] * sign[j * K + u]) << (8 * (u % 4));
-    }
     const dkgh::Zl b = dkgh::zl_from_bytes_wide(&mag[j * K * 32], 32);
     uint8_t w[32];
     dkgh::zl_to_bytes(w, dkgh::zl_mul(b, R));
     memcpy(&hs[8 * j], w, 32);
   }
+  ctx->sdig_jsf = -1;
   h2d(ctx, dd, hd.data(), 4 * hd.size());
   h2d(ctx, dt, ht.data(), 2 * n);
   h2d(ctx, ds, hs.data(), 4 * hs.size());
+  h2d(ctx, de, hev.data(), 4 * hev.size());
   ctx->sdig_n = n;
   ctx->sdig_L = L;
   ctx->sdig_K = K;
+  ctx->sdig_jsf = (int)jsf;
 }
 
 void verify_device(dkg_ctx* ctx, size_t n, size_t t, const VerifySeg* segs, int nseg, bool timed,
@@ -499,7 +551,7 @@
   }
   const size_t groups = (D + 63) / 64, gw = 64 * nseg;
   const size_t npad = groups * gw;
-  const size_t U = choose_split(ctx, npad, n, N), L = split_len(npad, n, N, U, ctx->combine_mode != 1), W = U * npad;
+  const size_t U = choose_split(ctx, npad, n, N), L = split_len(npad, n, N, U, short_kind(ctx)), W = U * npad;
   const size_t Lr = last_piece_len(N, U, L);
   const bool whole = ctx->step_mode == 1 || ((ctx->step_mode == 0 || ctx->step_mode == 3) && stepping_whole_pays(npad, U, L, Lr));
   const bool step_ilp = use_ilp(ctx, false);
@@ -512,7 +564,10 @@
   uint32_t* e0 = buf<uint32_t>(ctx, "v.binom0", PTB * L * W);
   uint32_t* e1 = buf<uint32_t>(ctx, "v.binom1", PTB * L * W);
   uint32_t* eT = buf<uint32_t>(ctx, "v.binomT", PTB * L * W);
-  uint32_t* R = buf<uint32_t>(ctx, "v.R", PTB * W * n);
+  const bool short_mult = U > 1 && U <= (ctx->addend_mode == 0 ? SHORT_MAX : 4) && ctx->combine_mode != 1;
+  const bool jsf = short_mult && short_kind(ctx) == SM_JSF && jsf_built(U) && (uint64_t)npad * n < (1ull << 32);
+  const size_t WP = jsf ? (U + 2 * (U / 2)) * npad : W;
+  uint32_t* R = buf<uint32_t>(ctx, "v.R", PTB * WP * n);
   uint32_t *sa = nullptr, *sb = nullptr;
   if (L > 512) {
     sa = buf<uint32_t>(ctx, "v.step_a", PTB * W * n);
@@ -520,16 +575,15 @@
   }
   const int8_t* ydig = nullptr;
   const int16_t* ytop = nullptr;
-  const uint32_t *sdig = nullptr, *sscale = nullptr;
+  const uint32_t *sdig = nullptr, *sscale = nullptr, *sev = nullptr;
   const int16_t* stop = nullptr;
-  const bool short_mult = U > 1 && U <= (ctx->addend_mode == 0 ? SHORT_MAX : 4) && ctx->combine_mode != 1;
   uint32_t* sflags = ctx->step_formula == 0
                          ? buf<uint32_t>(ctx, "v.sflags", 4 * dkgk::stepping_flag_words(npad, U)) : nullptr;
   ctx->last_step_flags = sflags;
   ctx->last_step_flag_words = sflags ? dkgk::stepping_flag_words(npad, U) : 0;
-  uint32_t* Aff = short_mult && ctx->addend_mode == 0 ? buf<uint32_t>(ctx, "v.Aff", 4 * AFFP_WORDS_H * W * n) : nullptr;
-  uint32_t* Rz = Aff ? buf<uint32_t>(ctx, "v.Rz", 40 * W * n) : nullptr;
-  if (short_mult) split_short(ctx, n, L, U, &sdig, &stop, &sscale);
+  uint32_t* Aff = short_mult && ctx->addend_mode == 0 ? buf<uint32_t>(ctx, "v.Aff", 4 * AFFP_WORDS_H * WP * n) : nullptr;
+  uint32_t* Rz = Aff ? buf<uint32_t>(ctx, "v.Rz", 40 * WP * n) : nullptr;
+  if (short_mult) split_short(ctx, n, L, U, jsf, &sdig, &stop, &sscale, &sev);
   else if (U > 1) split_digits(ctx, n, L, &ydig, &ytop);
   ctx->last_combine = U > 1 ? (short_mult ? 2 : 1) : 0;
   ctx->last_R = R;
@@ -631,7 +685,12 @@
               Rz ? Rz + c0 * n * 10 : nullptr, tail_a, tail_b))
       throw Fail{DKG_E_ARG};
     if (tm) HCK(hipEventRecord(ctx->pev[2], st));
-    if (short_mult && Aff) {
+    if (jsf) {
+      dkgk::pair_sums(w, npad, U, n, R + c0 * n * PT_WORDS_H, Rz + c0 * n * 10, st);
+      dkgk::affine_pieces(w, npad, U + 2 * (U / 2), n, R + c0 * n * PT_WORDS_H, Aff + c0 * n * AFFP_WORDS_H, st,
+                          Rz + c0 * n * 10);
+      dkgk::combine_short_jsf(w, npad, U, n, sdig, stop, sev, Aff + c0 * n * AFFP_WORDS_H, R + c0 * n * PT_WORDS_H, st);
+    } else if (short_mult && Aff) {
       dkgk::affine_pieces(w, npad, U, n, R + c0 * n * PT_WORDS_H, Aff + c0 * n * AFFP_WORDS_H, st, Rz + c0 * n * 10);
       dkgk::combine_short_aff(w, npad, U, n, sdig, stop, Aff + c0 * n * AFFP_WORDS_H, R + c0 * n * PT_WORDS_H, st);
     } else if (short_mult) dkgk::combine_short(w, npad, U, n, sdig, stop, R + c0 * n * PT_WORDS_H, st);
@@ -2174,7 +2233,7 @@
 int dkg_ctx_last_split(const dkg_ctx* ctx) { return ctx ? ctx->last_split : 0; }
 size_t dkg_ctx_last_split_len(const dkg_ctx* ctx) { return ctx ? ctx->last_split_len : 0; }
 int dkg_ctx_set_combine(dkg_ctx* ctx, int mode) {
-  if (!ctx || mode < 0 || mode > 2) return DKG_E_ARG;
+  if (!ctx || mode < 0 || mode > 3) return DKG_E_ARG;
   ctx->combine_mode = mode;
   return DKG_OK;
 }
@@ -2210,9 +2269,36 @@
   try {
     std::vector<uint8_t> m;
     std::vector<int8_t> sg;
-    short_vectors(n, L, (size_t)pieces, m, sg);
+    short_vectors(n, L, (size_t)pieces, m, sg, jsf_built((size_t)pieces));
     memcpy(mag, m.data(), m.size());
     memcpy(sign, sg.data(), sg.size());
+  } catch (const std::exception&) {
+    return DKG_E_NOMEM;
+  }
+  return DKG_OK;
+}
+int dkg_jsf_digits(const uint8_t a[32], const uint8_t b[32], int8_t da[256], int8_t db[256], int16_t* top) {
+  if (!a || !b || !da || !db || !top) return DKG_E_ARG;
+  return dkgh::jsf_digits(a, b, da, db, top) ? DKG_OK : DKG_E_ARG;
+}
+int dkg_split_digits(size_t n, size_t L, int pieces, int mode, int8_t* digits, int16_t* top) {
+  if (!n || !L || pieces < 2 || pieces > (int)SHORT_MAX || mode < 0 || mode > 3 || mode == 1 || !digits || !top)
+    return DKG_E_ARG;
+  try {
+    const size_t K = (size_t)pieces;
+    const bool jsf = mode != 3 && jsf_built(K);
+    std::vector<uint8_t> m;
+    std::vector<int8_t> sg;
+    short_vectors(n, L, K, m, sg, jsf);
+    std::vector<uint32_t> hd;
+    std::vector<int16_t> ht;
+    if (!short_digit_words(n, K, jsf, m, sg, hd, ht, nullptr)) return DKG_E_ARG;
+    for (size_t j = 0; j < n; j++) {
+      top[j] = ht[j];
+      for (size_t u = 0; u < K; u++)
+        for (size_t b = 0; b < 256; b++)
+          digits[(j * K + u) * 256 + b] = (int8_t)(hd[(u / 4) * 256 * n + 256 * j + b] >> (8 * (u % 4)));
+    }
   } catch (const std::exception&) {
     return DKG_E_NOMEM;
   }
diff --git a/include/dkg_amd.h b/include/dkg_amd.h
--- a/include/dkg_amd.h
+++ b/include/dkg_amd.h
@@ -46,6 +46,8 @@
 long long dkg_ctx_stepping_redos(dkg_ctx *ctx);
 int dkg_ctx_binomial_reruns(dkg_ctx *ctx);
 int dkg_split_multipliers(size_t n, size_t L, int pieces, uint8_t *mag, int8_t *sign);
+int dkg_jsf_digits(const uint8_t a[32], const uint8_t b[32], int8_t da[256], int8_t db[256], int16_t *top);
+int dkg_split_digits(size_t n, size_t L, int pieces, int mode, int8_t *digits, int16_t *top);
 int dkg_device_count(void);
 int dkg_ctx_clock_probe(dkg_ctx *ctx, unsigned iters, double *sclk_mhz, double *busy_ms);
 int dkg_device_pci_bus_id(int device, char *buf, int len);
```

After: 13.34 million verified shares/s (median of 6 runs). +1.5%, better.
